# 0xPARC/plonkathon

Measured on NVIDIA H100. Metric: plonk_proofs_per_s_2^20_gates, higher is better.
Workload: dtype u256 (BN254 Fr/Fq integers, 8x32-bit Montgomery limbs)

## Files before the change

### include/plonk_b200.h

```cpp
#ifndef PLONK_B200_H
#define PLONK_B200_H
#include <stddef.h>
#include <stdint.h>

#ifdef __cplusplus
extern "C" {
#endif

typedef struct pb200_ctx pb200_ctx;
typedef struct pb200_srs pb200_srs;
typedef struct pb200_prover pb200_prover;
typedef struct pb200_transcript pb200_transcript;

const char* pb200_last_error(void);
const char* pb200_version(void);
int pb200_ctx_create(int device, void* cuda_stream, pb200_ctx** out);
void pb200_ctx_destroy(pb200_ctx* ctx);
int pb200_ctx_sync(pb200_ctx* ctx);
uint64_t pb200_ctx_launches(pb200_ctx* ctx);
int pb200_ctx_timing(pb200_ctx* ctx, int enable);
int pb200_ctx_timing_read(pb200_ctx* ctx, int category, double* total_ms, uint64_t* count);
void* pb200_ctx_stream(pb200_ctx* ctx);

int pb200_fr_to_mont(pb200_ctx* ctx, const void* d_in, void* d_out, uint64_t n);
int pb200_fr_from_mont(pb200_ctx* ctx, const void* d_in, void* d_out, uint64_t n);

int pb200_fr_vec_op(pb200_ctx* ctx, int op, const void* d_a, const void* d_b, const uint8_t* h_scalar, void* d_out,
                    uint64_t n, uint64_t shift);

int pb200_fr_ntt(pb200_ctx* ctx, const void* d_in, void* d_out, unsigned log_n, int inverse);
int pb200_fr_ntt_host(pb200_ctx* ctx, const uint8_t* h_in, uint8_t* h_out, unsigned log_n, int inverse);

int pb200_fr_ntt_decimated(pb200_ctx* ctx, const void* d_in, void* d_out, unsigned log_m, int inverse, uint64_t stride,
                           uint64_t offset);

int pb200_fr_coset_extend(pb200_ctx* ctx, const void* d_in, void* d_out, unsigned log_n, const uint8_t* h_offset);
int pb200_fr_coset_extend_host(pb200_ctx* ctx, const uint8_t* h_in, uint8_t* h_out, unsigned log_n,
                               const uint8_t* h_offset);
int pb200_fr_coset_to_coeffs(pb200_ctx* ctx, const void* d_in, void* d_out, unsigned log_n, const uint8_t* h_offset);
int pb200_fr_coset_to_coeffs_host(pb200_ctx* ctx, const uint8_t* h_in, uint8_t* h_out, unsigned log_n,
                                  const uint8_t* h_offset);
int pb200_fr_barycentric_eval(pb200_ctx* ctx, const void* d_vals, unsigned log_n, const uint8_t* h_x, uint8_t* h_out);
int pb200_fr_barycentric_eval_host(pb200_ctx* ctx, const uint8_t* h_vals, unsigned log_n, const uint8_t* h_x,
                                   uint8_t* h_out);

int pb200_g1_msm(pb200_ctx* ctx, const void* d_points, const void* d_scalars, uint64_t n, uint8_t* h_out_xy,
                 int* is_identity);
int pb200_g1_msm_host(pb200_ctx* ctx, const uint8_t* h_points, const uint8_t* h_scalars, uint64_t n,
                      uint8_t* h_out_xy, int* is_identity);

int pb200_srs_create(pb200_ctx* ctx, const uint8_t* h_points, uint64_t n, int precompute, pb200_srs** out);
int pb200_srs_generate(pb200_ctx* ctx, const uint8_t* h_tau, uint64_t n, int precompute, pb200_srs** out);
int pb200_srs_generate_lagrange(pb200_ctx* ctx, const uint8_t* h_tau, uint64_t n, int precompute, pb200_srs** out);
int pb200_srs_export(pb200_ctx* ctx, pb200_srs* srs, uint8_t* h_points, uint64_t first, uint64_t count);
void pb200_srs_destroy(pb200_srs* srs);
uint64_t pb200_srs_size(pb200_srs* srs);
int pb200_srs_commit_lagrange(pb200_ctx* ctx, pb200_srs* srs, const void* d_values, unsigned log_n,
                              uint8_t* h_out_xy, int* is_identity);
int pb200_srs_commit_lagrange_host(pb200_ctx* ctx, pb200_srs* srs, const uint8_t* h_values, unsigned log_n,
                                   uint8_t* h_out_xy, int* is_identity);
int pb200_srs_commit_coeffs(pb200_ctx* ctx, pb200_srs* srs, const void* d_coeffs, uint64_t m, int coeffs_montgomery,
                            uint8_t* h_out_xy, int* is_identity);
int pb200_srs_commit_coeffs_host(pb200_ctx* ctx, pb200_srs* srs, const uint8_t* h_coeffs, uint64_t m,
                                 uint8_t* h_out_xy, int* is_identity);

int pb200_prover_create(pb200_ctx* ctx, pb200_srs* srs, unsigned log_n, const uint8_t* const* h_pk,
                        pb200_prover** out);
int pb200_prover_create_custom(pb200_ctx* ctx, pb200_srs* srs, unsigned log_n, const uint8_t* const* h_pk,
                               unsigned n_custom, const uint8_t* h_exps, const uint8_t* const* h_custom,
                               pb200_prover** out);
void pb200_prover_destroy(pb200_prover* p);
int pb200_prover_prove(pb200_prover* p, const uint8_t* h_A, const uint8_t* h_B, const uint8_t* h_C,
                       const uint8_t* h_public, uint64_t n_public, uint8_t* h_proof768);
int pb200_prover_prove_device(pb200_prover* p, const void* d_A, const void* d_B, const void* d_C,
                              const uint8_t* h_public, uint64_t n_public, uint8_t* h_proof768);
int pb200_prover_round1(pb200_prover* p, const uint8_t* h_A, const uint8_t* h_B, const uint8_t* h_C,
                        const uint8_t* h_public, uint64_t n_public, uint8_t* h_abc_xy );
int pb200_prover_round2(pb200_prover* p, const uint8_t* beta, const uint8_t* gamma, uint8_t* h_z_xy);
int pb200_prover_round3(pb200_prover* p, const uint8_t* alpha, const uint8_t* fft_cofactor,
                        uint8_t* h_t_xy );
int pb200_prover_round4(pb200_prover* p, const uint8_t* zeta, uint8_t* h_evals );
int pb200_prover_round5(pb200_prover* p, const uint8_t* v, uint8_t* h_w_xy );

int pb200_prover_read_vector(pb200_prover* p, int which, void* d_out);
int pb200_prover_set_zk(pb200_prover* p, int enable, const uint8_t* h_blinders);
int pb200_prover_serialize(pb200_prover* p, uint8_t* h_proof768);

int pb200_prover_set_lookup(pb200_prover* p, const uint8_t* h_qk, const uint8_t* h_t1, const uint8_t* h_t2,
                            const uint8_t* h_t3, uint64_t table_rows);
int pb200_prover_round_lookup(pb200_prover* p, const uint8_t* eta, uint8_t* h_fh_xy );
int pb200_prover_round2_lookup(pb200_prover* p, const uint8_t* beta, const uint8_t* gamma, const uint8_t* delta,
                               const uint8_t* epsilon, uint8_t* h_zz2_xy );
int pb200_prover_round4_lookup(pb200_prover* p, const uint8_t* zeta, uint8_t* h_evals );
int pb200_prover_prove_lookup(pb200_prover* p, const uint8_t* h_A, const uint8_t* h_B, const uint8_t* h_C,
                              const uint8_t* h_public, uint64_t n_public, uint8_t* h_proof1216);
int pb200_prover_serialize_lookup(pb200_prover* p, uint8_t* h_proof1216);

int pb200_comm_unique_id(uint8_t* out128);
int pb200_comm_init(pb200_ctx* ctx, const uint8_t* id128, int rank, int world);
int pb200_comm_info(pb200_ctx* ctx, int* rank, int* world, uint64_t* collectives, uint64_t* bytes_received);
int pb200_fr_ntt_sharded(pb200_ctx* ctx, const void* d_in, void* d_out, unsigned log_n, int inverse);
int pb200_srs_commit_coeffs_sharded(pb200_ctx* ctx, pb200_srs* srs, const void* d_coeffs, uint64_t m,
                                    int coeffs_montgomery, uint8_t* h_out_xy, int* is_identity);
int pb200_prover_create_sharded(pb200_ctx* ctx, pb200_srs* srs, unsigned log_n, const uint8_t* const* h_pk,
                                pb200_prover** out);
int pb200_prover_create_custom_sharded(pb200_ctx* ctx, pb200_srs* srs, unsigned log_n, const uint8_t* const* h_pk,
                                       unsigned n_custom, const uint8_t* h_exps, const uint8_t* const* h_custom,
                                       pb200_prover** out);
int pb200_srs_commit_partial(pb200_ctx* ctx, pb200_srs* srs, const void* d_coeffs, uint64_t first, uint64_t count,
                             uint32_t bucket_lo, uint32_t bucket_hi, int coeffs_montgomery, uint8_t* h_xyzz128);
int pb200_srs_bucket_count(pb200_srs* srs, uint32_t* out);
int pb200_g1_combine_partials_host(const uint8_t* h_xyzz, unsigned count, uint8_t* h_out_xy, int* is_identity);
int pb200_g1_join_bucket_shards_host(const uint8_t* h_sr, unsigned world, unsigned sets, uint32_t nloc, uint8_t* h_out_xy,
                                     int* is_identity);

int pb200_transcript_create(const uint8_t* label, size_t label_len, pb200_transcript** out);
void pb200_transcript_destroy(pb200_transcript* t);
int pb200_transcript_append_message(pb200_transcript* t, const uint8_t* label, size_t label_len,
                                    const uint8_t* msg, size_t msg_len);
int pb200_transcript_challenge_bytes(pb200_transcript* t, const uint8_t* label, size_t label_len, uint8_t* out,
                                     size_t n);
int pb200_transcript_get_and_append_challenge(pb200_transcript* t, const uint8_t* label, size_t label_len,
                                              uint8_t* out_le32);

int pb200_pairing_check(const uint8_t* h_g1, const uint8_t* h_g1_identity, const uint8_t* h_g2,
                        const uint8_t* h_g2_identity, unsigned count, int* ok);
int pb200_g2_mul(const uint8_t* h_point, const uint8_t* h_scalar_le32, uint8_t* h_out, int* is_identity);
int pb200_g2_add(const uint8_t* h_p, int p_identity, const uint8_t* h_q, int q_identity, uint8_t* h_out,
                 int* is_identity);

int pb200_bench_modmul(pb200_ctx* ctx, int field , uint64_t threads, uint32_t iters, float* ms_out);

#ifdef __cplusplus
}
#endif
#endif
```

### plonkathon_b200/_lib.py

```python
from __future__ import annotations

import ctypes
import os
import threading

_HERE = os.path.dirname(os.path.abspath(__file__))
LIB_PATH = os.environ.get("PB200_LIB") or os.path.join(_HERE, "libplonk_b200.so")

c_u8p = ctypes.POINTER(ctypes.c_uint8)


class PlonkB200Error(RuntimeError):
    pass


def _load():
    if not os.path.exists(LIB_PATH):
        raise PlonkB200Error(
            "libplonk_b200.so is not built (%s); run `python -c 'import __graft_entry__ as g; g.build()'`"
            % LIB_PATH)
    lib = ctypes.CDLL(LIB_PATH)
    V, I, U, U64 = ctypes.c_void_p, ctypes.c_int, ctypes.c_uint, ctypes.c_uint64
    P = ctypes.POINTER
    sig = {
        "pb200_last_error": (ctypes.c_char_p, []),
        "pb200_version": (ctypes.c_char_p, []),
        "pb200_ctx_create": (I, [I, V, P(V)]),
        "pb200_ctx_destroy": (None, [V]),
        "pb200_ctx_sync": (I, [V]),
        "pb200_ctx_launches": (U64, [V]),
        "pb200_ctx_stream": (V, [V]),
        "pb200_ctx_timing": (I, [V, I]),
        "pb200_ctx_timing_read": (I, [V, I, P(ctypes.c_double), P(U64)]),
        "pb200_fr_to_mont": (I, [V, V, V, U64]),
        "pb200_fr_from_mont": (I, [V, V, V, U64]),
        "pb200_fr_ntt": (I, [V, V, V, U, I]),
        "pb200_fr_ntt_host": (I, [V, V, V, U, I]),
        "pb200_fr_ntt_decimated": (I, [V, V, V, U, I, U64, U64]),
        "pb200_fr_ntt_sharded": (I, [V, V, V, U, I]),
        "pb200_fr_vec_op": (I, [V, I, V, V, V, V, U64, U64]),
        "pb200_prover_read_vector": (I, [V, I, V]),
        "pb200_comm_unique_id": (I, [V]),
        "pb200_comm_init": (I, [V, V, I, I]),
        "pb200_comm_info": (I, [V, P(I), P(I), P(U64), P(U64)]),
        "pb200_srs_commit_coeffs_sharded": (I, [V, V, V, U64, I, V, P(I)]),
        "pb200_prover_create_sharded": (I, [V, V, U, V, P(V)]),
        "pb200_srs_commit_partial": (I, [V, V, V, U64, U64, U, U, I, V]),
        "pb200_srs_bucket_count": (I, [V, P(U)]),
        "pb200_g1_join_bucket_shards_host": (I, [V, U, U, U, V, P(I)]),
        "pb200_fr_coset_extend": (I, [V, V, V, U, V]),
        "pb200_fr_coset_extend_host": (I, [V, V, V, U, V]),
        "pb200_fr_coset_to_coeffs": (I, [V, V, V, U, V]),
        "pb200_fr_coset_to_coeffs_host": (I, [V, V, V, U, V]),
        "pb200_fr_barycentric_eval": (I, [V, V, U, V, V]),
        "pb200_fr_barycentric_eval_host": (I, [V, V, U, V, V]),
        "pb200_g1_msm": (I, [V, V, V, U64, V, P(I)]),
        "pb200_g1_msm_host": (I, [V, V, V, U64, V, P(I)]),
        "pb200_srs_create": (I, [V, V, U64, I, P(V)]),
        "pb200_srs_generate": (I, [V, V, U64, I, P(V)]),
        "pb200_srs_generate_lagrange": (I, [V, V, U64, I, P(V)]),
        "pb200_srs_export": (I, [V, V, V, U64, U64]),
        "pb200_srs_destroy": (None, [V]),
        "pb200_srs_size": (U64, [V]),
        "pb200_srs_commit_lagrange": (I, [V, V, V, U, V, P(I)]),
        "pb200_srs_commit_lagrange_host": (I, [V, V, V, U, V, P(I)]),
        "pb200_srs_commit_coeffs_host": (I, [V, V, V, U64, V, P(I)]),
        "pb200_srs_commit_coeffs": (I, [V, V, V, U64, I, V, P(I)]),
        "pb200_prover_create": (I, [V, V, U, V, P(V)]),
        "pb200_prover_create_custom": (I, [V, V, U, V, U, V, V, P(V)]),
        "pb200_prover_create_custom_sharded": (I, [V, V, U, V, U, V, V, P(V)]),
        "pb200_prover_destroy": (None, [V]),
        "pb200_prover_prove": (I, [V, V, V, V, V, U64, V]),
        "pb200_prover_prove_device": (I, [V, V, V, V, V, U64, V]),
        "pb200_prover_round1": (I, [V, V, V, V, V, U64, V]),
        "pb200_prover_round2": (I, [V, V, V, V]),
        "pb200_prover_round3": (I, [V, V, V, V]),
        "pb200_prover_round4": (I, [V, V, V]),
        "pb200_prover_round5": (I, [V, V, V]),
        "pb200_prover_serialize": (I, [V, V]),
        "pb200_prover_set_zk": (I, [V, I, V]),
        "pb200_prover_set_lookup": (I, [V, V, V, V, V, U64]),
        "pb200_prover_round_lookup": (I, [V, V, V]),
        "pb200_prover_round2_lookup": (I, [V, V, V, V, V, V]),
        "pb200_prover_round4_lookup": (I, [V, V, V]),
        "pb200_prover_prove_lookup": (I, [V, V, V, V, V, U64, V]),
        "pb200_prover_serialize_lookup": (I, [V, V]),
        "pb200_g1_combine_partials_host": (I, [V, U, V, P(I)]),
        "pb200_transcript_create": (I, [V, ctypes.c_size_t, P(V)]),
        "pb200_transcript_destroy": (None, [V]),
        "pb200_transcript_append_message": (I, [V, V, ctypes.c_size_t, V, ctypes.c_size_t]),
        "pb200_transcript_challenge_bytes": (I, [V, V, ctypes.c_size_t, V, ctypes.c_size_t]),
        "pb200_transcript_get_and_append_challenge": (I, [V, V, ctypes.c_size_t, V]),
        "pb200_pairing_check": (I, [V, V, V, V, U, P(I)]),
        "pb200_g2_mul": (I, [V, V, V, P(I)]),
        "pb200_g2_add": (I, [V, I, V, I, V, P(I)]),
        "pb200_bench_modmul": (I, [V, I, U64, U, P(ctypes.c_float)]),
    }
    for name, (res, args) in sig.items():
        fn = getattr(lib, name)
        fn.restype = res
        fn.argtypes = args
    return lib, tuple(sig)


_lock = threading.Lock()
_lib = None
EXPORTS = ()


def lib():
    global _lib, EXPORTS
    with _lock:
        if _lib is None:
            _lib, EXPORTS = _load()
    return _lib


def check(rc):
    if rc != 0:
        raise PlonkB200Error(lib().pb200_last_error().decode())


class Context:

    def __init__(self, device: int = 0, stream: int | None = None):
        h = ctypes.c_void_p()
        check(lib().pb200_ctx_create(device, ctypes.c_void_p(stream), ctypes.byref(h)))
        self.handle = h
        self.device = device

    def sync(self):
        check(lib().pb200_ctx_sync(self.handle))

    @property
    def launches(self) -> int:
        return int(lib().pb200_ctx_launches(self.handle))

    @property
    def stream(self) -> int:
        return int(lib().pb200_ctx_stream(self.handle) or 0)

    def close(self):
        if self.handle:
            lib().pb200_ctx_destroy(self.handle)
            self.handle = None

    def __del__(self):
        try:
            self.close()
        except Exception:
            pass


_default_ctx = None


def default_context() -> Context:
    global _default_ctx
    if _default_ctx is None:
        _default_ctx = Context(int(os.environ.get("LOCAL_RANK", "0")))
    return _default_ctx
```

### plonkathon_b200/csrc/capi.cu

```cuda
#include "../../include/plonk_b200.h"

#include <cstring>

#include "common.cuh"
#include "comm.cuh"
#include "msm_bucket.cuh"
#include "prover.cuh"
#include "pairing.cuh"
#include "transcript.cuh"

namespace pb200 {
void ntt_run(Context* ctx, const Fr* in, Fr* out, int log_n, bool inverse, uint64_t n_in, const Fr* in_scale,
             const Fr* out_scale);
void launch_powers(Context* ctx, Fr* out, uint64_t n, const Fr& base, const Fr& scale);
Fr fr_from_u64(uint64_t x);
void ntt_run_strided(Context* ctx, const Fr* in, Fr* out, int log_n, bool inverse, uint64_t n_in,
                     const Fr* in_scale, const Fr* out_scale, uint64_t in_mul, uint64_t in_add);
void ntt_sharded(Context* ctx, const Fr* const* in, Fr* const* out, int count, int log_n, bool inverse);
void fr_to_mont(Context* ctx, const Fr* in, Fr* out, uint64_t n);
void fr_from_mont(Context* ctx, const Fr* in, Fr* out, uint64_t n);
void fr_vec_op(Context* ctx, int op, const Fr* a, const Fr* b, const Fr& scalar_canonical, Fr* out, uint64_t n,
               uint64_t shift);
void barycentric_eval(Context* ctx, const Fr* d_vals, int log_n, const Fr& x_mont, Fr* h_out);
float bench_modmul(Context* ctx, int field, uint64_t threads, uint32_t iters);
struct Srs;
Srs* srs_create(Context* ctx, const uint8_t* h_points, uint64_t n, int precompute);
void srs_destroy(Srs* s);
Srs* srs_generate(Context* ctx, const Fr& tau_canonical, uint64_t n, int precompute);
Srs* srs_generate_lagrange(Context* ctx, const Fr& tau_canonical, uint64_t n, int precompute);
void srs_export(Context* ctx, Srs* srs, uint8_t* h_points, uint64_t first, uint64_t count);
void srs_msm(Context* ctx, Srs* srs, const Fr* d_scalars, uint64_t m, bool scalars_mont, uint8_t* out_xy, int* is_identity);
uint64_t srs_size(Srs* s);
uint32_t msm_default_window(uint64_t n, bool fixed_base);
void msm_run(Context* ctx, const G1Affine* points, uint64_t n, const Fr* scalars, bool scalars_mont, uint32_t c,
             bool fixed_base, uint64_t point_stride, uint8_t* out_xy, int* is_identity);
void affine_to_mont(Context* ctx, const G1Affine* in, G1Affine* out, uint64_t n);
Prover* prover_create(Context* ctx, Srs* srs, int log_n, const uint8_t* const* h_pk, int n_custom,
                      const uint8_t* h_exps, const uint8_t* const* h_custom, bool sharded);
void prover_destroy(Prover* p);
void prover_prove(Prover* P, const uint8_t* hA, const uint8_t* hB, const uint8_t* hC, const uint8_t* h_public,
                  uint64_t n_public, uint8_t* out768, bool wires_on_device);
void prover_round1(Prover* P, const uint8_t* hA, const uint8_t* hB, const uint8_t* hC, const uint8_t* h_public,
                   uint64_t n_public, bool wires_on_device);
void prover_round2(Prover* P, const Fr& beta_c, const Fr& gamma_c);
void prover_round3(Prover* P, const Fr& alpha_c, const Fr& cofactor_c);
void prover_round4(Prover* P, const Fr& zeta_c);
void prover_round5(Prover* P, const Fr& v_c);
void prover_serialize(const Prover* P, uint8_t* out768);
void prover_set_zk(Prover* P, bool enable, const uint8_t* h_blinders);
void prover_set_lookup(Prover* P, const uint8_t* h_qk, const uint8_t* const* h_tab, uint64_t rows);
void prover_round_lookup(Prover* P, const Fr& eta_c);
void prover_round2_lookup(Prover* P, const Fr& beta_c, const Fr& gamma_c, const Fr& delta_c, const Fr& epsilon_c);
void prover_round4_lookup(Prover* P, const Fr& zeta_c);
void prover_prove_lookup(Prover* P, const uint8_t* hA, const uint8_t* hB, const uint8_t* hC, const uint8_t* h_public,
                         uint64_t n_public, uint8_t* out1216);
void prover_serialize_lookup(const Prover* P, uint8_t* out1216);
void g1_combine_partials_host(const G1XYZZ* parts, uint32_t count, uint8_t* out_xy, int* is_identity);
void host_join_bucket_shards(const SR* all, uint32_t world, uint32_t sets, uint32_t nloc, G1XYZZ* out);
void host_join_bucket_shards_strided(const SR* all, uint32_t world, uint32_t sets, G1XYZZ* out);
}

using namespace pb200;

static thread_local std::string g_err;

#define PB_API_BEGIN try {
#define PB_API_END                        \
  return 0;                               \
  }                                       \
  catch (const std::exception& e) {       \
    g_err = e.what();                     \
    return 1;                             \
  }                                       \
  catch (...) {                           \
    g_err = "unknown error";              \
    return 1;                             \
  }

static Context* C(pb200_ctx* c) { return reinterpret_cast<Context*>(c); }

#define PB_NOT_LOOKUP(P, entry)                                                                       \
  PB_CHECK(!(P)->lk, "this prover has a lookup argument: its proofs have 1216 bytes; use " entry)

struct DeviceGuard {
  int prev = -1;
  explicit DeviceGuard(const Context* c) {
    int cur = -1;
    cudaGetDevice(&cur);
    if (cur != c->device) { cudaSetDevice(c->device); prev = cur; }
  }
  ~DeviceGuard() { if (prev >= 0) cudaSetDevice(prev); }
};
#define PB_ON_CTX(c) DeviceGuard guard__(c)

static Fr load_fr_canonical(const uint8_t* h) {
  Fr a;
  memcpy(a.v, h, 32);
  Fr m = Fr::modulus();
  bool lt = false;
  for (int i = 7; i >= 0; i--) {
    if (a.v[i] != m.v[i]) { lt = a.v[i] < m.v[i]; break; }
  }
  PB_CHECK(lt, "Fr value not reduced below the modulus");
  return a;
}

extern "C" {

const char* pb200_last_error(void) { return g_err.c_str(); }
const char* pb200_version(void) { return "plonk_b200 0.1 (sm_90a)"; }

int pb200_ctx_create(int device, void* cuda_stream, pb200_ctx** out) {
  PB_API_BEGIN
  int count = 0;
  cudaError_t e = cudaGetDeviceCount(&count);
  PB_CHECK(e == cudaSuccess && count > 0, "no CUDA device: libplonk_b200 has no CPU fallback");
  PB_CHECK(device >= 0 && device < count, "bad device ordinal");
  PB_CUDA(cudaSetDevice(device));
  auto ctx = std::make_unique<Context>();
  ctx->device = device;
  cudaDeviceProp prop;
  PB_CUDA(cudaGetDeviceProperties(&prop, device));
  ctx->sm_count = prop.multiProcessorCount;
  if (cuda_stream) {
    ctx->stream = reinterpret_cast<cudaStream_t>(cuda_stream);
  } else {
    PB_CUDA(cudaStreamCreateWithFlags(&ctx->stream, cudaStreamNonBlocking));
    ctx->own_stream = true;
  }
  *out = reinterpret_cast<pb200_ctx*>(ctx.release());
  PB_API_END
}

void pb200_ctx_destroy(pb200_ctx* ctx) {
  if (!ctx) return;
  cudaSetDevice(C(ctx)->device);
  cudaStreamSynchronize(C(ctx)->stream);
  delete C(ctx);
}

int pb200_ctx_sync(pb200_ctx* ctx) {
  PB_API_BEGIN PB_ON_CTX(C(ctx));
  PB_CUDA(cudaStreamSynchronize(C(ctx)->stream));
  PB_API_END
}

uint64_t pb200_ctx_launches(pb200_ctx* ctx) { return C(ctx)->launches; }

int pb200_ctx_timing(pb200_ctx* ctx, int enable) {
  PB_API_BEGIN PB_ON_CTX(C(ctx));
  Context* c = C(ctx);
  PB_CUDA(cudaStreamSynchronize(c->stream));
  for (auto& v : c->timed) {
    for (auto& pr : v) { cudaEventDestroy(pr.first); cudaEventDestroy(pr.second); }
    v.clear();
  }
  c->timing = enable != 0;
  PB_API_END
}
int pb200_ctx_timing_read(pb200_ctx* ctx, int category, double* total_ms, uint64_t* count) {
  PB_API_BEGIN PB_ON_CTX(C(ctx));
  Context* c = C(ctx);
  PB_CHECK(category >= 0 && category < 4, "bad timing category");
  PB_CUDA(cudaStreamSynchronize(c->stream));
  double t = 0;
  for (auto& pr : c->timed[category]) {
    float ms = 0;
    PB_CUDA(cudaEventElapsedTime(&ms, pr.first, pr.second));
    t += ms;
  }
  *total_ms = t;
  *count = c->timed[category].size();
  PB_API_END
}
void* pb200_ctx_stream(pb200_ctx* ctx) { return (void*)C(ctx)->stream; }

int pb200_fr_to_mont(pb200_ctx* ctx, const void* d_in, void* d_out, uint64_t n) {
  PB_API_BEGIN PB_ON_CTX(C(ctx));
  fr_to_mont(C(ctx), (const Fr*)d_in, (Fr*)d_out, n);
  PB_API_END
}
int pb200_fr_from_mont(pb200_ctx* ctx, const void* d_in, void* d_out, uint64_t n) {
  PB_API_BEGIN PB_ON_CTX(C(ctx));
  fr_from_mont(C(ctx), (const Fr*)d_in, (Fr*)d_out, n);
  PB_API_END
}

int pb200_fr_vec_op(pb200_ctx* ctx, int op, const void* d_a, const void* d_b, const uint8_t* h_scalar, void* d_out,
                    uint64_t n, uint64_t shift) {
  PB_API_BEGIN PB_ON_CTX(C(ctx));
  Fr s = Fr::zero();
  if (h_scalar) s = load_fr_canonical(h_scalar);
  PB_CHECK(op < 4 ? d_b != nullptr : true, "missing second operand");
  fr_vec_op(C(ctx), op, (const Fr*)d_a, (const Fr*)d_b, s, (Fr*)d_out, n, shift);
  PB_API_END
}

int pb200_fr_ntt(pb200_ctx* ctx, const void* d_in, void* d_out, unsigned log_n, int inverse) {
  PB_API_BEGIN PB_ON_CTX(C(ctx));
  ntt_run(C(ctx), (const Fr*)d_in, (Fr*)d_out, (int)log_n, inverse != 0, (uint64_t)1 << log_n, nullptr, nullptr);
  PB_API_END
}

int pb200_fr_ntt_decimated(pb200_ctx* ctx, const void* d_in, void* d_out, unsigned log_m, int inverse, uint64_t stride,
                           uint64_t offset) {
  PB_API_BEGIN PB_ON_CTX(C(ctx));
  PB_CHECK(stride >= 1, "bad stride");
  ntt_run_strided(C(ctx), (const Fr*)d_in, (Fr*)d_out, (int)log_m, inverse != 0, (uint64_t)1 << log_m, nullptr, nullptr,
                  stride, offset);
  PB_API_END
}
int pb200_fr_ntt_sharded(pb200_ctx* ctx, const void* d_in, void* d_out, unsigned log_n, int inverse) {
  PB_API_BEGIN PB_ON_CTX(C(ctx));
  const Fr* in = (const Fr*)d_in;
  Fr* out = (Fr*)d_out;
  ntt_sharded(C(ctx), &in, &out, 1, (int)log_n, inverse != 0);
  PB_API_END
}

int pb200_comm_unique_id(uint8_t* out128) {
  PB_API_BEGIN
  comm_unique_id(out128);
  PB_API_END
}
int pb200_comm_init(pb200_ctx* ctx, const uint8_t* id128, int rank, int world) {
  PB_API_BEGIN PB_ON_CTX(C(ctx));
  Context* c = C(ctx);
  PB_CHECK(!c->comm, "this context already has a communicator");
  c->comm = comm_create(id128, rank, world);
  PB_API_END
}
int pb200_comm_info(pb200_ctx* ctx, int* rank, int* world, uint64_t* collectives, uint64_t* bytes_received) {
  PB_API_BEGIN
  Context* c = C(ctx);
  *rank = c->comm ? c->comm->rank : 0;
  *world = c->comm ? c->comm->world : 1;
  *collectives = c->comm ? c->comm->collectives : 0;
  *bytes_received = c->comm ? c->comm->bytes_gathered : 0;
  PB_API_END
}

struct HostStage {
  Context* ctx;
  DevBuf in, out;
  HostStage(Context* c, const uint8_t* h_in, size_t in_bytes, size_t out_bytes) : ctx(c), in(in_bytes), out(out_bytes) {
    if (in_bytes) PB_CUDA(cudaMemcpyAsync(in.p, h_in, in_bytes, cudaMemcpyHostToDevice, ctx->stream));
  }
  void finish(uint8_t* h_out, size_t bytes) {
    PB_CUDA(cudaMemcpyAsync(h_out, out.p, bytes, cudaMemcpyDeviceToHost, ctx->stream));
    PB_CUDA(cudaStreamSynchronize(ctx->stream));
  }
};

int pb200_fr_ntt_host(pb200_ctx* ctx, const uint8_t* h_in, uint8_t* h_out, unsigned log_n, int inverse) {
  PB_API_BEGIN PB_ON_CTX(C(ctx));
  size_t bytes = ((size_t)1 << log_n) * 32;
  HostStage st(C(ctx), h_in, bytes, bytes);
  ntt_run(C(ctx), st.in.as<Fr>(), st.out.as<Fr>(), (int)log_n, inverse != 0, (uint64_t)1 << log_n, nullptr, nullptr);
  st.finish(h_out, bytes);
  PB_API_END
}

static void coset_extend(Context* ctx, const Fr* d_in, Fr* d_out, int log_n, const uint8_t* h_offset) {
  uint64_t n = (uint64_t)1 << log_n;
  Fr off = fp_to_mont(load_fr_canonical(h_offset));
  DevBuf coeffs(n * 32), powers(n * 32);
  ntt_run(ctx, d_in, coeffs.as<Fr>(), log_n, true, n, nullptr, nullptr);
  launch_powers(ctx, powers.as<Fr>(), n, off, Fr::one());
  ntt_run(ctx, coeffs.as<Fr>(), d_out, log_n + 2, false, n, powers.as<Fr>(), nullptr);
  PB_CUDA(cudaStreamSynchronize(ctx->stream));
}

static void coset_to_coeffs(Context* ctx, const Fr* d_in, Fr* d_out, int log_n, const uint8_t* h_offset) {
  uint64_t n = (uint64_t)1 << log_n;
  Fr off = fp_to_mont(load_fr_canonical(h_offset));
  Fr inv = fp_inv(off);
  DevBuf powers(n * 32);
  launch_powers(ctx, powers.as<Fr>(), n, inv, Fr::one());
  ntt_run(ctx, d_in, d_out, log_n, true, n, nullptr, powers.as<Fr>());
  PB_CUDA(cudaStreamSynchronize(ctx->stream));
}

int pb200_fr_coset_extend(pb200_ctx* ctx, const void* d_in, void* d_out, unsigned log_n, const uint8_t* h_offset) {
  PB_API_BEGIN PB_ON_CTX(C(ctx));
  coset_extend(C(ctx), (const Fr*)d_in, (Fr*)d_out, (int)log_n, h_offset);
  PB_API_END
}
int pb200_fr_coset_extend_host(pb200_ctx* ctx, const uint8_t* h_in, uint8_t* h_out, unsigned log_n,
                               const uint8_t* h_offset) {
  PB_API_BEGIN PB_ON_CTX(C(ctx));
  size_t bytes = ((size_t)1 << log_n) * 32;
  HostStage st(C(ctx), h_in, bytes, bytes * 4);
  coset_extend(C(ctx), st.in.as<Fr>(), st.out.as<Fr>(), (int)log_n, h_offset);
  st.finish(h_out, bytes * 4);
  PB_API_END
}
int pb200_fr_coset_to_coeffs(pb200_ctx* ctx, const void* d_in, void* d_out, unsigned log_n, const uint8_t* h_offset) {
  PB_API_BEGIN PB_ON_CTX(C(ctx));
  coset_to_coeffs(C(ctx), (const Fr*)d_in, (Fr*)d_out, (int)log_n, h_offset);
  PB_API_END
}
int pb200_fr_coset_to_coeffs_host(pb200_ctx* ctx, const uint8_t* h_in, uint8_t* h_out, unsigned log_n,
                                  const uint8_t* h_offset) {
  PB_API_BEGIN PB_ON_CTX(C(ctx));
  size_t bytes = ((size_t)1 << log_n) * 32;
  HostStage st(C(ctx), h_in, bytes, bytes);
  coset_to_coeffs(C(ctx), st.in.as<Fr>(), st.out.as<Fr>(), (int)log_n, h_offset);
  st.finish(h_out, bytes);
  PB_API_END
}

int pb200_fr_barycentric_eval(pb200_ctx* ctx, const void* d_vals, unsigned log_n, const uint8_t* h_x, uint8_t* h_out) {
  PB_API_BEGIN PB_ON_CTX(C(ctx));
  Fr x = fp_to_mont(load_fr_canonical(h_x));
  Fr r;
  barycentric_eval(C(ctx), (const Fr*)d_vals, (int)log_n, x, &r);
  memcpy(h_out, r.v, 32);
  PB_API_END
}
int pb200_fr_barycentric_eval_host(pb200_ctx* ctx, const uint8_t* h_vals, unsigned log_n, const uint8_t* h_x,
                                   uint8_t* h_out) {
  PB_API_BEGIN PB_ON_CTX(C(ctx));
  size_t bytes = ((size_t)1 << log_n) * 32;
  HostStage st(C(ctx), h_vals, bytes, 0);
  Fr x = fp_to_mont(load_fr_canonical(h_x));
  Fr r;
  barycentric_eval(C(ctx), st.in.as<Fr>(), (int)log_n, x, &r);
  memcpy(h_out, r.v, 32);
  PB_API_END
}

int pb200_g1_msm(pb200_ctx* ctx, const void* d_points, const void* d_scalars, uint64_t n, uint8_t* h_out_xy,
                 int* is_identity) {
  PB_API_BEGIN PB_ON_CTX(C(ctx));
  PB_CHECK(n > 0, "ec_lincomb of an empty list (the reference raises ValueError, curve.py:93)");
  Context* c = C(ctx);
  DevBuf mont(n * sizeof(G1Affine));
  affine_to_mont(c, (const G1Affine*)d_points, mont.as<G1Affine>(), n);
  msm_run(c, mont.as<G1Affine>(), n, (const Fr*)d_scalars, false, msm_default_window(n, false), false, 0, h_out_xy,
          is_identity);
  PB_API_END
}

int pb200_g1_msm_host(pb200_ctx* ctx, const uint8_t* h_points, const uint8_t* h_scalars, uint64_t n,
                      uint8_t* h_out_xy, int* is_identity) {
  PB_API_BEGIN PB_ON_CTX(C(ctx));
  PB_CHECK(n > 0, "ec_lincomb of an empty list (the reference raises ValueError, curve.py:93)");
  Context* c = C(ctx);
  DevBuf pts(n * 64), sc(n * 32);
  PB_CUDA(cudaMemcpyAsync(pts.p, h_points, n * 64, cudaMemcpyHostToDevice, c->stream));
  PB_CUDA(cudaMemcpyAsync(sc.p, h_scalars, n * 32, cudaMemcpyHostToDevice, c->stream));
  int rc = pb200_g1_msm(ctx, pts.p, sc.p, n, h_out_xy, is_identity);
  if (rc) throw Error(g_err);
  PB_API_END
}

int pb200_srs_create(pb200_ctx* ctx, const uint8_t* h_points, uint64_t n, int precompute, pb200_srs** out) {
  PB_API_BEGIN PB_ON_CTX(C(ctx));
  PB_CHECK(n > 0, "empty SRS");
  *out = reinterpret_cast<pb200_srs*>(srs_create(C(ctx), h_points, n, precompute));
  PB_API_END
}
int pb200_srs_generate(pb200_ctx* ctx, const uint8_t* h_tau, uint64_t n, int precompute, pb200_srs** out) {
  PB_API_BEGIN PB_ON_CTX(C(ctx));
  PB_CHECK(n > 0, "empty SRS");
  *out = reinterpret_cast<pb200_srs*>(srs_generate(C(ctx), load_fr_canonical(h_tau), n, precompute));
  PB_API_END
}
int pb200_srs_generate_lagrange(pb200_ctx* ctx, const uint8_t* h_tau, uint64_t n, int precompute, pb200_srs** out) {
  PB_API_BEGIN PB_ON_CTX(C(ctx));
  PB_CHECK(n > 0, "empty SRS");
  *out = reinterpret_cast<pb200_srs*>(srs_generate_lagrange(C(ctx), load_fr_canonical(h_tau), n, precompute));
  PB_API_END
}
int pb200_srs_commit_coeffs_host(pb200_ctx* ctx, pb200_srs* srs, const uint8_t* h_coeffs, uint64_t m,
                                 uint8_t* h_out_xy, int* is_identity) {
  PB_API_BEGIN PB_ON_CTX(C(ctx));
  HostStage st(C(ctx), h_coeffs, (size_t)m * 32, 0);
  srs_msm(C(ctx), reinterpret_cast<Srs*>(srs), (const Fr*)st.in.p, m, false, h_out_xy, is_identity);
  PB_API_END
}
int pb200_srs_export(pb200_ctx* ctx, pb200_srs* srs, uint8_t* h_points, uint64_t first, uint64_t count) {
  PB_API_BEGIN PB_ON_CTX(C(ctx));
  srs_export(C(ctx), reinterpret_cast<Srs*>(srs), h_points, first, count);
  PB_API_END
}
void pb200_srs_destroy(pb200_srs* srs) { srs_destroy(reinterpret_cast<Srs*>(srs)); }
uint64_t pb200_srs_size(pb200_srs* srs) { return srs_size(reinterpret_cast<Srs*>(srs)); }

int pb200_srs_commit_lagrange(pb200_ctx* ctx, pb200_srs* srs, const void* d_values, unsigned log_n, uint8_t* h_out_xy,
                              int* is_identity) {
  PB_API_BEGIN PB_ON_CTX(C(ctx));
  Context* c = C(ctx);
  uint64_t n = (uint64_t)1 << log_n;
  PB_CHECK(n <= srs_size(reinterpret_cast<Srs*>(srs)), "Not enough powers in setup");
  DevBuf coeffs(n * 32);
  ntt_run(c, (const Fr*)d_values, coeffs.as<Fr>(), (int)log_n, true, n, nullptr, nullptr);
  srs_msm(c, reinterpret_cast<Srs*>(srs), coeffs.as<Fr>(), n, false, h_out_xy, is_identity);
  PB_API_END
}
int pb200_srs_commit_lagrange_host(pb200_ctx* ctx, pb200_srs* srs, const uint8_t* h_values, unsigned log_n,
                                   uint8_t* h_out_xy, int* is_identity) {
  PB_API_BEGIN PB_ON_CTX(C(ctx));
  size_t bytes = ((size_t)1 << log_n) * 32;
  HostStage st(C(ctx), h_values, bytes, 0);
  int rc = pb200_srs_commit_lagrange(ctx, srs, st.in.p, log_n, h_out_xy, is_identity);
  if (rc) throw Error(g_err);
  PB_API_END
}
int pb200_srs_commit_coeffs(pb200_ctx* ctx, pb200_srs* srs, const void* d_coeffs, uint64_t m, int coeffs_montgomery,
                            uint8_t* h_out_xy, int* is_identity) {
  PB_API_BEGIN PB_ON_CTX(C(ctx));
  srs_msm(C(ctx), reinterpret_cast<Srs*>(srs), (const Fr*)d_coeffs, m, coeffs_montgomery != 0, h_out_xy, is_identity);
  PB_API_END
}

int pb200_prover_create(pb200_ctx* ctx, pb200_srs* srs, unsigned log_n, const uint8_t* const* h_pk,
                        pb200_prover** out) {
  return pb200_prover_create_custom(ctx, srs, log_n, h_pk, 0, nullptr, nullptr, out);
}
int pb200_prover_create_sharded(pb200_ctx* ctx, pb200_srs* srs, unsigned log_n, const uint8_t* const* h_pk,
                                pb200_prover** out) {
  return pb200_prover_create_custom_sharded(ctx, srs, log_n, h_pk, 0, nullptr, nullptr, out);
}
int pb200_prover_create_custom(pb200_ctx* ctx, pb200_srs* srs, unsigned log_n, const uint8_t* const* h_pk,
                               unsigned n_custom, const uint8_t* h_exps, const uint8_t* const* h_custom,
                               pb200_prover** out) {
  PB_API_BEGIN PB_ON_CTX(C(ctx));
  *out = reinterpret_cast<pb200_prover*>(prover_create(C(ctx), reinterpret_cast<Srs*>(srs), (int)log_n, h_pk,
                                                       (int)n_custom, h_exps, h_custom, false));
  PB_API_END
}
int pb200_prover_create_custom_sharded(pb200_ctx* ctx, pb200_srs* srs, unsigned log_n, const uint8_t* const* h_pk,
                                       unsigned n_custom, const uint8_t* h_exps, const uint8_t* const* h_custom,
                                       pb200_prover** out) {
  PB_API_BEGIN PB_ON_CTX(C(ctx));
  *out = reinterpret_cast<pb200_prover*>(prover_create(C(ctx), reinterpret_cast<Srs*>(srs), (int)log_n, h_pk,
                                                       (int)n_custom, h_exps, h_custom, true));
  PB_API_END
}
void pb200_prover_destroy(pb200_prover* p) { prover_destroy(reinterpret_cast<Prover*>(p)); }

int pb200_prover_prove(pb200_prover* p, const uint8_t* h_A, const uint8_t* h_B, const uint8_t* h_C,
                       const uint8_t* h_public, uint64_t n_public, uint8_t* h_proof768) {
  PB_API_BEGIN PB_ON_CTX(reinterpret_cast<Prover*>(p)->ctx);
  PB_NOT_LOOKUP(reinterpret_cast<Prover*>(p), "pb200_prover_prove_lookup");
  prover_prove(reinterpret_cast<Prover*>(p), h_A, h_B, h_C, h_public, n_public, h_proof768, false);
  PB_API_END
}
int pb200_prover_prove_device(pb200_prover* p, const void* d_A, const void* d_B, const void* d_C,
                              const uint8_t* h_public, uint64_t n_public, uint8_t* h_proof768) {
  PB_API_BEGIN PB_ON_CTX(reinterpret_cast<Prover*>(p)->ctx);
  PB_NOT_LOOKUP(reinterpret_cast<Prover*>(p), "pb200_prover_prove_lookup (wires in host memory)");
  prover_prove(reinterpret_cast<Prover*>(p), (const uint8_t*)d_A, (const uint8_t*)d_B, (const uint8_t*)d_C, h_public,
               n_public, h_proof768, true);
  PB_API_END
}
int pb200_prover_round1(pb200_prover* p, const uint8_t* h_A, const uint8_t* h_B, const uint8_t* h_C,
                        const uint8_t* h_public, uint64_t n_public, uint8_t* h_abc_xy) {
  PB_API_BEGIN PB_ON_CTX(reinterpret_cast<Prover*>(p)->ctx);
  Prover* P = reinterpret_cast<Prover*>(p);
  prover_round1(P, h_A, h_B, h_C, h_public, n_public, false);
  memcpy(h_abc_xy, P->proof.pts[0], 3 * 64);
  PB_API_END
}
int pb200_prover_round2(pb200_prover* p, const uint8_t* beta, const uint8_t* gamma, uint8_t* h_z_xy) {
  PB_API_BEGIN PB_ON_CTX(reinterpret_cast<Prover*>(p)->ctx);
  Prover* P = reinterpret_cast<Prover*>(p);
  PB_NOT_LOOKUP(P, "pb200_prover_round2_lookup");
  prover_round2(P, load_fr_canonical(beta), load_fr_canonical(gamma));
  memcpy(h_z_xy, P->proof.pts[3], 64);
  PB_API_END
}
int pb200_prover_round3(pb200_prover* p, const uint8_t* alpha, const uint8_t* fft_cofactor, uint8_t* h_t_xy) {
  PB_API_BEGIN PB_ON_CTX(reinterpret_cast<Prover*>(p)->ctx);
  Prover* P = reinterpret_cast<Prover*>(p);
  prover_round3(P, load_fr_canonical(alpha), load_fr_canonical(fft_cofactor));
  memcpy(h_t_xy, P->proof.pts[4], 3 * 64);
  PB_API_END
}
int pb200_prover_round4(pb200_prover* p, const uint8_t* zeta, uint8_t* h_evals) {
  PB_API_BEGIN PB_ON_CTX(reinterpret_cast<Prover*>(p)->ctx);
  Prover* P = reinterpret_cast<Prover*>(p);
  PB_NOT_LOOKUP(P, "pb200_prover_round4_lookup");
  prover_round4(P, load_fr_canonical(zeta));
  memcpy(h_evals, P->proof.evals[0], 6 * 32);
  PB_API_END
}
int pb200_prover_round5(pb200_prover* p, const uint8_t* v, uint8_t* h_w_xy) {
  PB_API_BEGIN PB_ON_CTX(reinterpret_cast<Prover*>(p)->ctx);
  Prover* P = reinterpret_cast<Prover*>(p);
  prover_round5(P, load_fr_canonical(v));
  memcpy(h_w_xy, P->proof.pts[7], 2 * 64);
  PB_API_END
}

int pb200_prover_read_vector(pb200_prover* p, int which, void* d_out) {
  PB_API_BEGIN PB_ON_CTX(reinterpret_cast<Prover*>(p)->ctx);
  Prover* P = reinterpret_cast<Prover*>(p);
  const Fr* src = nullptr;
  switch (which) {
    case 0: case 1: case 2: case 3: src = P->lag[which].as<Fr>(); break;
    case 4: src = P->pi_lag.as<Fr>(); break;
    case 5: case 6: case 7:
      PB_CHECK(!P->zk, "T1, T2, T3 are not n-coefficient vectors in zero-knowledge mode (the blinded pieces have n + 1, "
                       "n + 1 and n + 6 coefficients)");
      src = P->tq.as<Fr>() + (uint64_t)(which - 5) * P->n;
      break;
    default: PB_CHECK(false, "unknown prover vector");
  }
  fr_from_mont(P->ctx, src, (Fr*)d_out, P->n);
  PB_CUDA(cudaStreamSynchronize(P->ctx->stream));
  PB_API_END
}
int pb200_prover_set_zk(pb200_prover* p, int enable, const uint8_t* h_blinders) {
  PB_API_BEGIN PB_ON_CTX(reinterpret_cast<Prover*>(p)->ctx);
  prover_set_zk(reinterpret_cast<Prover*>(p), enable != 0, h_blinders);
  PB_API_END
}
int pb200_prover_serialize(pb200_prover* p, uint8_t* h_proof768) {
  PB_API_BEGIN PB_ON_CTX(reinterpret_cast<Prover*>(p)->ctx);
  PB_NOT_LOOKUP(reinterpret_cast<Prover*>(p), "pb200_prover_serialize_lookup");
  prover_serialize(reinterpret_cast<Prover*>(p), h_proof768);
  PB_API_END
}
int pb200_prover_set_lookup(pb200_prover* p, const uint8_t* h_qk, const uint8_t* h_t1, const uint8_t* h_t2,
                            const uint8_t* h_t3, uint64_t table_rows) {
  PB_API_BEGIN PB_ON_CTX(reinterpret_cast<Prover*>(p)->ctx);
  const uint8_t* tab[3] = {h_t1, h_t2, h_t3};
  prover_set_lookup(reinterpret_cast<Prover*>(p), h_qk, tab, table_rows);
  PB_API_END
}
int pb200_prover_round_lookup(pb200_prover* p, const uint8_t* eta, uint8_t* h_fh_xy) {
  PB_API_BEGIN PB_ON_CTX(reinterpret_cast<Prover*>(p)->ctx);
  Prover* P = reinterpret_cast<Prover*>(p);
  prover_round_lookup(P, load_fr_canonical(eta));
  memcpy(h_fh_xy, P->lk_pts[0], 3 * 64);
  PB_API_END
}
int pb200_prover_round2_lookup(pb200_prover* p, const uint8_t* beta, const uint8_t* gamma, const uint8_t* delta,
                               const uint8_t* epsilon, uint8_t* h_zz2_xy) {
  PB_API_BEGIN PB_ON_CTX(reinterpret_cast<Prover*>(p)->ctx);
  Prover* P = reinterpret_cast<Prover*>(p);
  prover_round2_lookup(P, load_fr_canonical(beta), load_fr_canonical(gamma), load_fr_canonical(delta),
                       load_fr_canonical(epsilon));
  memcpy(h_zz2_xy, P->proof.pts[3], 64);
  memcpy(h_zz2_xy + 64, P->lk_pts[3], 64);
  PB_API_END
}
int pb200_prover_round4_lookup(pb200_prover* p, const uint8_t* zeta, uint8_t* h_evals) {
  PB_API_BEGIN PB_ON_CTX(reinterpret_cast<Prover*>(p)->ctx);
  Prover* P = reinterpret_cast<Prover*>(p);
  prover_round4_lookup(P, load_fr_canonical(zeta));
  memcpy(h_evals, P->proof.evals[0], 6 * 32);
  memcpy(h_evals + 6 * 32, P->lk_evals[0], 6 * 32);
  PB_API_END
}
int pb200_prover_prove_lookup(pb200_prover* p, const uint8_t* h_A, const uint8_t* h_B, const uint8_t* h_C,
                              const uint8_t* h_public, uint64_t n_public, uint8_t* h_proof1216) {
  PB_API_BEGIN PB_ON_CTX(reinterpret_cast<Prover*>(p)->ctx);
  prover_prove_lookup(reinterpret_cast<Prover*>(p), h_A, h_B, h_C, h_public, n_public, h_proof1216);
  PB_API_END
}
int pb200_prover_serialize_lookup(pb200_prover* p, uint8_t* h_proof1216) {
  PB_API_BEGIN PB_ON_CTX(reinterpret_cast<Prover*>(p)->ctx);
  Prover* P = reinterpret_cast<Prover*>(p);
  PB_CHECK(P->lk, "this prover has no lookup table: use pb200_prover_serialize (768 bytes)");
  prover_serialize_lookup(P, h_proof1216);
  PB_API_END
}
int pb200_g1_combine_partials_host(const uint8_t* h_xyzz, unsigned count, uint8_t* h_out_xy, int* is_identity) {
  PB_API_BEGIN
  std::vector<G1XYZZ> parts(count);
  memcpy(parts.data(), h_xyzz, (size_t)count * sizeof(G1XYZZ));
  g1_combine_partials_host(parts.data(), count, h_out_xy, is_identity);
  PB_API_END
}

int pb200_srs_commit_partial(pb200_ctx* ctx, pb200_srs* srs, const void* d_coeffs, uint64_t first, uint64_t count,
                             uint32_t bucket_lo, uint32_t bucket_hi, int coeffs_montgomery, uint8_t* h_xyzz128) {
  PB_API_BEGIN PB_ON_CTX(C(ctx));
  const Fr* sc = (const Fr*)d_coeffs;
  G1XYZZ part;
  srs_msm_batch_partial(C(ctx), reinterpret_cast<Srs*>(srs), &sc, 1, first, count, bucket_lo, bucket_hi,
                        coeffs_montgomery != 0, &part);
  memcpy(h_xyzz128, &part, sizeof(part));
  PB_API_END
}
int pb200_srs_bucket_count(pb200_srs* srs, uint32_t* out) {
  PB_API_BEGIN
  *out = srs_bucket_count(reinterpret_cast<Srs*>(srs));
  PB_API_END
}
int pb200_srs_commit_coeffs_sharded(pb200_ctx* ctx, pb200_srs* srs, const void* d_coeffs, uint64_t m,
                                    int coeffs_montgomery, uint8_t* h_out_xy, int* is_identity) {
  PB_API_BEGIN PB_ON_CTX(C(ctx));
  const Fr* sc = (const Fr*)d_coeffs;
  srs_msm_batch_sharded(C(ctx), reinterpret_cast<Srs*>(srs), &sc, 1, m, coeffs_montgomery != 0, h_out_xy, is_identity);
  PB_API_END
}
int pb200_g1_join_bucket_shards_host(const uint8_t* h_sr, unsigned world, unsigned sets, uint32_t nloc, uint8_t* h_out_xy,
                                     int* is_identity) {
  PB_API_BEGIN
  std::vector<SR> all((size_t)world * sets);
  memcpy(all.data(), h_sr, all.size() * sizeof(SR));
  std::vector<G1XYZZ> ws(sets);
  if (nloc == 0) host_join_bucket_shards_strided(all.data(), world, sets, ws.data());
  else host_join_bucket_shards(all.data(), world, sets, nloc, ws.data());
  for (unsigned k = 0; k < sets; k++) g1_combine_partials_host(&ws[k], 1, h_out_xy + 64 * k, is_identity + k);
  PB_API_END
}

int pb200_transcript_create(const uint8_t* label, size_t label_len, pb200_transcript** out) {
  PB_API_BEGIN
  *out = reinterpret_cast<pb200_transcript*>(new Transcript(std::string((const char*)label, label_len)));
  PB_API_END
}
void pb200_transcript_destroy(pb200_transcript* t) { delete reinterpret_cast<Transcript*>(t); }
int pb200_transcript_append_message(pb200_transcript* t, const uint8_t* label, size_t label_len, const uint8_t* msg,
                                    size_t msg_len) {
  PB_API_BEGIN
  reinterpret_cast<Transcript*>(t)->append_message(std::string((const char*)label, label_len), msg, msg_len);
  PB_API_END
}
int pb200_transcript_challenge_bytes(pb200_transcript* t, const uint8_t* label, size_t label_len, uint8_t* out,
                                     size_t n) {
  PB_API_BEGIN
  reinterpret_cast<Transcript*>(t)->challenge_bytes(std::string((const char*)label, label_len), out, n);
  PB_API_END
}
int pb200_transcript_get_and_append_challenge(pb200_transcript* t, const uint8_t* label, size_t label_len,
                                              uint8_t* out_le32) {
  PB_API_BEGIN
  Fr f = reinterpret_cast<Transcript*>(t)->get_and_append_challenge(std::string((const char*)label, label_len));
  memcpy(out_le32, f.v, 32);
  PB_API_END
}

static Fq load_fq_canonical(const uint8_t* h) {
  Fq a;
  memcpy(a.v, h, 32);
  Fq m = Fq::modulus();
  bool lt = false;
  for (int i = 7; i >= 0; i--) {
    if (a.v[i] != m.v[i]) { lt = a.v[i] < m.v[i]; break; }
  }
  PB_CHECK(lt, "Fq value not reduced below the modulus");
  return fp_to_mont(a);
}
static G2Affine load_g2(const uint8_t* h, bool inf) {
  G2Affine q;
  q.inf = inf;
  q.x = {load_fq_canonical(h), load_fq_canonical(h + 32)};
  q.y = {load_fq_canonical(h + 64), load_fq_canonical(h + 96)};
  PB_CHECK(inf || g2_on_curve(q), "G2 point is not on the twist curve");
  return q;
}
static void store_g2(const G2Affine& q, uint8_t* out, int* is_identity) {
  *is_identity = q.inf ? 1 : 0;
  memset(out, 0, 128);
  if (q.inf) return;
  const Fq c[4] = {fp_from_mont(q.x.a), fp_from_mont(q.x.b), fp_from_mont(q.y.a), fp_from_mont(q.y.b)};
  for (int k = 0; k < 4; k++) memcpy(out + 32 * k, c[k].v, 32);
}
static const Bn254Pairing& pairing_engine() {
  static const Bn254Pairing engine;
  return engine;
}

int pb200_pairing_check(const uint8_t* h_g1, const uint8_t* h_g1_identity, const uint8_t* h_g2,
                        const uint8_t* h_g2_identity, unsigned count, int* ok) {
  PB_API_BEGIN
  std::vector<G1Host> ps(count);
  std::vector<G2Affine> qs(count);
  const Fq three = fq_small(3);
  for (unsigned i = 0; i < count; i++) {
    ps[i].inf = h_g1_identity && h_g1_identity[i];
    if (!ps[i].inf) {
      ps[i].x = load_fq_canonical(h_g1 + 64 * i);
      ps[i].y = load_fq_canonical(h_g1 + 64 * i + 32);
      PB_CHECK(fp_sqr(ps[i].y) == fp_add(fp_mul(fp_sqr(ps[i].x), ps[i].x), three), "G1 point is not on the curve");
    }
    qs[i] = load_g2(h_g2 + 128 * i, h_g2_identity && h_g2_identity[i]);
  }
  *ok = pairing_engine().product_is_one(ps, qs) ? 1 : 0;
  PB_API_END
}
int pb200_g2_mul(const uint8_t* h_point, const uint8_t* h_scalar_le32, uint8_t* h_out, int* is_identity) {
  PB_API_BEGIN
  G2Affine p = load_g2(h_point, false);
  uint32_t k[8];
  memcpy(k, h_scalar_le32, 32);
  store_g2(g2_mul(p, k), h_out, is_identity);
  PB_API_END
}
int pb200_g2_add(const uint8_t* h_p, int p_identity, const uint8_t* h_q, int q_identity, uint8_t* h_out,
                 int* is_identity) {
  PB_API_BEGIN
  store_g2(g2_add(load_g2(h_p, p_identity != 0), load_g2(h_q, q_identity != 0)), h_out, is_identity);
  PB_API_END
}

int pb200_bench_modmul(pb200_ctx* ctx, int field, uint64_t threads, uint32_t iters, float* ms_out) {
  PB_API_BEGIN PB_ON_CTX(C(ctx));
  *ms_out = bench_modmul(C(ctx), field, threads, iters);
  PB_API_END
}

}
```

### plonkathon_b200/csrc/host_selftest.cpp

```cpp
#include "field.cuh"
#include "curve.cuh"
#include "msm_digits.cuh"
#include "modinv.cuh"
#include "msm_bucket.cuh"
#include "msm_sort.cuh"
#include "ntt_shard.cuh"
#include <algorithm>
#include <vector>
#include <cstring>
using namespace pb200;

template <class F> static F ld(const uint32_t* p) { F r; memcpy(r.v, p, 32); return r; }
template <class F> static void st(uint32_t* p, const F& a) { memcpy(p, a.v, 32); }

extern "C" {
int hs_field_op(int field, int op, const uint32_t* a, const uint32_t* b, uint32_t* out) {
#define RUN(F)                                                   \
  {                                                              \
    F x = ld<F>(a), y = ld<F>(b), r;                             \
    switch (op) {                                                \
      case 0: r = fp_add(x, y); break;                           \
      case 1: r = fp_sub(x, y); break;                           \
      case 2: r = fp_mul(x, y); break;                           \
      case 3: r = fp_neg(x); break;                              \
      case 4: r = fp_inv(x); break;                              \
      case 5: r = fp_to_mont(x); break;                          \
      case 6: r = fp_from_mont(x); break;                        \
      case 7: r = fp_dbl(x); break;                              \
      case 8: r = fp_sqr(x); break;                              \
      case 9: r = fp_inv_gcd(x); break;                          \
      case 10: r = fp_inv_plain_gcd(x); break;                   \
      case 11: r = fp_mul_lazy(x, y); break;                     \
      case 12: r = fp_sqr_lazy(x); break;                        \
      case 13: r = fp_sub_lazy(x, y); break;                     \
      case 14: r = fp_neg_lazy(x); break;                        \
      case 15: r = fp_is_zero_lazy(x) ? F::one() : F::zero(); break; \
      default: return -1;                                        \
    }                                                            \
    st(out, r);                                                  \
  }
  if (field == 0) RUN(Fr) else RUN(Fq)
#undef RUN
  return 0;
}

int hs_field_mul2(int field, const uint32_t* a, const uint32_t* b, const uint32_t* c, const uint32_t* d, uint32_t* out) {
  if (field == 0) st(out, fp_mul2_lazy(ld<Fr>(a), ld<Fr>(b), ld<Fr>(c), ld<Fr>(d)));
  else st(out, fp_mul2_lazy(ld<Fq>(a), ld<Fq>(b), ld<Fq>(c), ld<Fq>(d)));
  return 0;
}
}

static Fq ref_sqr(const Fq& a) { return fp_mul(a, a); }
static void ref_double(G1XYZZ& a) {
  if (a.is_inf()) return;
  Fq U = fp_dbl(a.Y), V = ref_sqr(U), W = fp_mul(U, V), S = fp_mul(a.X, V), M = ref_sqr(a.X);
  M = fp_add(fp_dbl(M), M);
  Fq X3 = fp_sub(ref_sqr(M), fp_dbl(S));
  a.Y = fp_sub(fp_mul(M, fp_sub(S, X3)), fp_mul(W, a.Y));
  a.X = X3;
  a.ZZ = fp_mul(V, a.ZZ);
  a.ZZZ = fp_mul(W, a.ZZZ);
}
static void ref_add_mixed(G1XYZZ& acc, const G1Affine& p) {
  if (acc.is_inf()) { acc = g1_from_affine(p); return; }
  Fq U2 = fp_mul(p.x, acc.ZZ), S2 = fp_mul(p.y, acc.ZZZ), Pd = fp_sub(U2, acc.X), Rd = fp_sub(S2, acc.Y);
  if (Pd.is_zero()) {
    if (Rd.is_zero()) { acc = g1_from_affine(p); ref_double(acc); }
    else acc = G1XYZZ::identity();
    return;
  }
  Fq PP = ref_sqr(Pd), PPP = fp_mul(Pd, PP), Q = fp_mul(acc.X, PP);
  Fq X3 = fp_sub(fp_sub(ref_sqr(Rd), PPP), fp_dbl(Q));
  acc.Y = fp_sub(fp_mul(Rd, fp_sub(Q, X3)), fp_mul(acc.Y, PPP));
  acc.X = X3;
  acc.ZZ = fp_mul(acc.ZZ, PP);
  acc.ZZZ = fp_mul(acc.ZZZ, PPP);
}
static void ref_add(G1XYZZ& acc, const G1XYZZ& q) {
  if (q.is_inf()) return;
  if (acc.is_inf()) { acc = q; return; }
  Fq U1 = fp_mul(acc.X, q.ZZ), U2 = fp_mul(q.X, acc.ZZ), S1 = fp_mul(acc.Y, q.ZZZ), S2 = fp_mul(q.Y, acc.ZZZ);
  Fq Pd = fp_sub(U2, U1), Rd = fp_sub(S2, S1);
  if (Pd.is_zero()) {
    if (Rd.is_zero()) ref_double(acc);
    else acc = G1XYZZ::identity();
    return;
  }
  Fq PP = ref_sqr(Pd), PPP = fp_mul(Pd, PP), Q = fp_mul(U1, PP);
  Fq X3 = fp_sub(fp_sub(ref_sqr(Rd), PPP), fp_dbl(Q));
  acc.Y = fp_sub(fp_mul(Rd, fp_sub(Q, X3)), fp_mul(S1, PPP));
  acc.X = X3;
  acc.ZZ = fp_mul(fp_mul(acc.ZZ, q.ZZ), PP);
  acc.ZZZ = fp_mul(fp_mul(acc.ZZZ, q.ZZZ), PPP);
}

extern "C" {
int hs_curve_op_ref(int op, const uint32_t* acc_in, const uint32_t* other, int other_inf, uint32_t* out) {
  G1XYZZ acc;
  memcpy(&acc, acc_in, sizeof(acc));
  if (op == 0 || op == 4) {
    G1Affine p;
    memcpy(&p.x, other, 32);
    memcpy(&p.y, other + 8, 32);
    if (!other_inf) ref_add_mixed(acc, p);
  } else if (op == 1 || op == 5) {
    G1XYZZ q;
    memcpy(&q, other, sizeof(q));
    ref_add(acc, q);
  } else if (op == 2) {
    ref_double(acc);
  } else {
    return -1;
  }
  memcpy(out, &acc, sizeof(acc));
  return 0;
}

int hs_small_dft(int log_g, const uint32_t* x, const uint32_t* tw, uint32_t* out) {
  DftTw t;
  for (int k = 0; k < 4; k++) t.w[k] = ld<Fr>(tw + 8 * k);
#define RUN_DFT(LG)                                                     \
  {                                                                     \
    Fr v[1 << LG];                                                      \
    for (int i = 0; i < (1 << LG); i++) v[i] = ld<Fr>(x + 8 * i);       \
    small_dft<LG>(v, t);                                                \
    for (int i = 0; i < (1 << LG); i++) st(out + 8 * i, v[i]);          \
  }
  switch (log_g) {
    case 1: RUN_DFT(1) break;
    case 2: RUN_DFT(2) break;
    case 3: RUN_DFT(3) break;
    default: return -1;
  }
#undef RUN_DFT
  return 0;
}

int hs_msm_digits(const uint32_t* scalar, uint32_t c, int32_t* digits, uint32_t* n_windows) {
  MsmGeom g;
  g.c = c;
  g.W = (256 + c - 1) / c;
  g.half = 1u << (c - 1);
  g.fixed_base = 0;
  g.point_stride = 0;
  g.batch = 1;
  g.lo = 0;
  g.nloc = g.half;
  g.own_log = 0;
  g.own_rank = 0;
  g.sets = g.W;
  g.nb = g.half * g.W;
  Fr s = ld<Fr>(scalar);
  DigitWalk dw(&s, 0, 0);
  for (uint32_t w = 0; w < g.W; w++) {
    uint32_t neg, d = dw.next(w, g, neg);
    digits[w] = neg ? -(int32_t)d : (int32_t)d;
  }
  *n_windows = g.W;
  return (int)dw.carry;
}

int hs_curve_op(int op, const uint32_t* acc_in, const uint32_t* other, int other_inf, uint32_t* out) {
  G1XYZZ acc;
  memcpy(&acc, acc_in, sizeof(acc));
  switch (op) {
    case 0: {
      G1Affine p;
      memcpy(&p.x, other, 32);
      memcpy(&p.y, other + 8, 32);
      if (!other_inf) g1_add_mixed(acc, p);
      break;
    }
    case 4: {
      G1Affine p;
      memcpy(&p.x, other, 32);
      memcpy(&p.y, other + 8, 32);
      if (!other_inf) g1_add_mixed_uniform(acc, p);
      break;
    }
    case 1: {
      G1XYZZ q;
      memcpy(&q, other, sizeof(q));
      g1_add(acc, q);
      break;
    }
    case 2: g1_double(acc); break;
    case 5: {
      G1XYZZ q;
      memcpy(&q, other, sizeof(q));
      g1_add_uniform(acc, q);
      break;
    }
    case 3: {
      G1Affine p;
      bool inf = g1_to_affine(acc, p);
      memcpy(out, &p.x, 32);
      memcpy(out + 8, &p.y, 32);
      return inf ? 1 : 0;
    }
    default: return -1;
  }
  memcpy(out, &acc, sizeof(acc));
  return 0;
}

}

static bool msm_geom(uint32_t n, uint32_t batch, uint32_t c, int fixed_base, uint32_t lo, uint32_t hi, MsmGeom& g) {
  g.c = c;
  g.W = (256 + c - 1) / c;
  g.half = 1u << (c - 1);
  g.fixed_base = fixed_base ? 1 : 0;
  g.point_stride = fixed_base ? n : 0;
  g.batch = batch;
  g.own_log = 0;
  g.own_rank = 0;
  if (hi >= 0xfffffff0u && hi != 0xffffffffu) {
    g.own_log = 0xffffffffu - hi;
    g.own_rank = lo;
    g.lo = 0;
    g.nloc = g.half >> g.own_log;
    if (!g.nloc || lo >= (1u << g.own_log)) return false;
  } else {
    if (hi > g.half) hi = g.half;
    if (lo >= hi) return false;
    g.lo = lo;
    g.nloc = hi - lo;
  }
  g.sets = fixed_base ? batch : g.W;
  g.nb = g.sets * g.nloc;
  return true;
}

static void host_scan(uint32_t* cnt, uint32_t len, uint32_t pad, uint32_t* off, uint32_t* max_out) {
  uint32_t run = 0, m = 0;
  for (uint32_t b = 0; b < len; b++) {
    off[b] = run;
    run += (cnt[b] + pad) & ~pad;
    m = std::max(m, cnt[b]);
    cnt[b] = 0;
  }
  off[len] = run;
  if (max_out) *max_out = m;
}

static void host_msm_sort(const MsmGeom& g, const std::vector<Fr>& sc, uint32_t n, uint32_t pad, uint32_t lb,
                          uint32_t T, uint32_t spb, uint32_t bin_nt, uint32_t chunk_nt, std::vector<uint32_t>& counts,
                          std::vector<uint32_t>& off, std::vector<uint32_t>& sorted) {
  const uint32_t nbins = ((g.nb - 1) >> lb) + 1;
  const uint32_t batch = g.fixed_base ? g.batch : 1;
  std::vector<uint32_t> bin_cnt(nbins, 0), bin_off(nbins + 1), chunk_first(nbins + 1);
  std::vector<SortEntry> binned((size_t)n * g.W * batch);
  counts.assign(g.nb + 1, 0);
  off.assign(g.nb + 1, 0);
  SortArgs a;
  for (uint32_t k = 0; k < 4; k++) a.sb.p[k] = k < batch ? sc.data() + (size_t)k * n : nullptr;
  a.n = n;
  a.from_mont = 0;
  a.g = g;
  a.lb = lb;
  a.nbins = nbins;
  a.T = T;
  a.bin_cnt = bin_cnt.data();
  a.bin_off = bin_off.data();
  a.binned = binned.data();
  a.chunk_first = chunk_first.data();
  a.counts = counts.data();
  a.offsets = off.data();
  a.sorted = nullptr;
  a.spb = spb;
  std::vector<uint32_t> sh_cnt(std::max(nbins, 1u << lb)), sh_loc(sh_cnt.size()), sh_base(sh_cnt.size()), runs;
  std::vector<SortEntry> bin_stage_buf((size_t)spb * g.W);
  std::vector<uint32_t> chunk_stage_buf(T);
  auto block_scan = [&](uint32_t len, uint32_t nt) {
    runs.assign(nt, 0);
    uint32_t run = 0;
    for (uint32_t t = 0; t < nt; t++) { runs[t] = run; run += scan_part_sum(sh_cnt.data(), len, t, nt); }
    return run;
  };
  const uint32_t bin_blocks = (n + spb - 1) / spb;
  for (uint32_t k = 0; k < batch; k++)
    for (uint32_t bx = 0; bx < bin_blocks; bx++) {
      for (uint32_t t = 0; t < bin_nt; t++) sort_zero(sh_cnt.data(), nbins, t, bin_nt);
      for (uint32_t t = 0; t < bin_nt; t++) bin_hist(a, bx, k, t, bin_nt, sh_cnt.data());
      for (uint32_t t = 0; t < bin_nt; t++) bin_flush(a, t, bin_nt, sh_cnt.data());
    }
  host_scan(bin_cnt.data(), nbins, 0, bin_off.data(), nullptr);
  for (uint32_t k = batch; k-- > 0;)
    for (uint32_t bx = bin_blocks; bx-- > 0;) {
      for (uint32_t t = 0; t < bin_nt; t++) sort_zero(sh_cnt.data(), nbins, t, bin_nt);
      for (uint32_t t = 0; t < bin_nt; t++) bin_hist(a, bx, k, t, bin_nt, sh_cnt.data());
      const uint32_t total = block_scan(nbins, bin_nt);
      for (uint32_t t = 0; t < bin_nt; t++)
        bin_reserve(a, t, bin_nt, runs[t], sh_cnt.data(), sh_loc.data(), sh_base.data());
      for (uint32_t t = 0; t < bin_nt; t++) bin_stage(a, bx, k, t, bin_nt, sh_cnt.data(), sh_loc.data(), bin_stage_buf.data());
      for (uint32_t t = 0; t < bin_nt; t++)
        bin_copy_out(a, t, bin_nt, total, sh_loc.data(), sh_base.data(), bin_stage_buf.data());
    }
  {
    std::vector<uint32_t> sums(256);
    for (uint32_t t = 0; t < 256; t++) sums[t] = chunk_map_sum(a, t);
    uint32_t run = 0;
    for (uint32_t t = 0; t < 256; t++) { const uint32_t s = sums[t]; sums[t] = run; run += s; }
    for (uint32_t t = 0; t < 256; t++) chunk_map_write(a, t, sums[t], run);
  }
  const uint32_t grid = 3;
  SortChunk ch;
  for (uint32_t bx = 0; bx < grid; bx++)
    for (uint32_t c = bx; chunk_locate(a, c, ch); c += grid) {
      for (uint32_t t = 0; t < chunk_nt; t++) sort_zero(sh_cnt.data(), ch.nkeys, t, chunk_nt);
      for (uint32_t t = 0; t < chunk_nt; t++) chunk_hist(a, ch, t, chunk_nt, sh_cnt.data());
      for (uint32_t t = 0; t < chunk_nt; t++) chunk_flush(a, ch, t, chunk_nt, sh_cnt.data());
    }
  host_scan(counts.data(), g.nb, pad, off.data(), &counts[g.nb]);
  sorted.assign(off[g.nb] + 2, PB_MSM_PAD);
  a.sorted = sorted.data();
  for (uint32_t bx = grid; bx-- > 0;)
    for (uint32_t c = bx; chunk_locate(a, c, ch); c += grid) {
      for (uint32_t t = 0; t < chunk_nt; t++) sort_zero(sh_cnt.data(), ch.nkeys, t, chunk_nt);
      for (uint32_t t = 0; t < chunk_nt; t++) chunk_hist(a, ch, t, chunk_nt, sh_cnt.data());
      const uint32_t total = block_scan(ch.nkeys, chunk_nt);
      for (uint32_t t = 0; t < chunk_nt; t++)
        chunk_reserve(a, ch, t, chunk_nt, runs[t], sh_cnt.data(), sh_loc.data(), sh_base.data());
      for (uint32_t t = 0; t < chunk_nt; t++) chunk_stage(a, ch, t, chunk_nt, sh_cnt.data(), sh_loc.data(), chunk_stage_buf.data());
      for (uint32_t t = 0; t < chunk_nt; t++)
        chunk_copy_out(a, ch, t, chunk_nt, sh_loc.data(), sh_base.data(), chunk_stage_buf.data());
      if (total != ch.hi - ch.lo) abort();
    }
}

extern "C" {
int hs_msm_sort(const uint32_t* scalars, uint32_t n, uint32_t batch, uint32_t c, int fixed_base, uint32_t lo,
                uint32_t hi, uint32_t pad, uint32_t lb, uint32_t T, uint32_t spb, uint32_t bin_nt, uint32_t chunk_nt,
                uint32_t* counts_out, uint32_t* off_out, uint32_t* sorted_out, uint32_t cap) {
  if (!n || !batch || batch > 4 || (!fixed_base && batch != 1) || c < 1 || c > 16 || !T || !bin_nt || !chunk_nt)
    return -1;
  MsmGeom g;
  if (!msm_geom(n, batch, c, fixed_base, lo, hi, g)) return -1;
  if (lb == 0xffffffffu) lb = sort_default_lb(g.nb);
  if (((g.nb - 1) >> lb) >= PB_SORT_MAX_BINS || (1u << lb) > PB_SORT_MAX_BIN_KEYS) return -1;
  if (!spb) spb = PB_SORT_BIN_STAGE / g.W;
  std::vector<Fr> sc((size_t)batch * n);
  for (size_t i = 0; i < sc.size(); i++) sc[i] = ld<Fr>(scalars + 8 * i);
  std::vector<uint32_t> counts, off, sorted;
  host_msm_sort(g, sc, n, pad ? 1 : 0, lb, T, spb, bin_nt, chunk_nt, counts, off, sorted);
  if (off[g.nb] > cap) return -1;
  memcpy(counts_out, counts.data(), counts.size() * 4);
  memcpy(off_out, off.data(), off.size() * 4);
  memcpy(sorted_out, sorted.data(), (size_t)off[g.nb] * 4);
  return (int)g.nb;
}

int hs_msm_pipeline(const uint32_t* points, uint32_t n, const uint32_t* scalars, uint32_t batch, uint32_t c,
                    int fixed_base, uint32_t lo, uint32_t hi, uint32_t B, uint32_t g0, uint32_t* out, uint8_t* out_inf) {
  if (!n || !batch || batch > 4 || (!fixed_base && batch != 1) || c < 1 || c > 16 || B < 2 || B > PB_AFF_BMAX) return -1;
  if (g0 < 2 || (g0 & (g0 - 1))) return -1;
  MsmGeom g;
  if (!msm_geom(n, batch, c, fixed_base, lo, hi, g)) return -1;
  std::vector<G1Affine> tab(fixed_base ? (size_t)g.W * n : n);
  for (uint32_t i = 0; i < n; i++) {
    tab[i].x = fp_to_mont(ld<Fq>(points + 16 * i));
    tab[i].y = fp_to_mont(ld<Fq>(points + 16 * i + 8));
  }
  if (fixed_base)
    for (uint32_t w = 1; w < g.W; w++)
      for (uint32_t i = 0; i < n; i++) {
        G1XYZZ a;
        g1_double_affine(a, tab[(size_t)(w - 1) * n + i]);
        for (uint32_t k = 1; k < c; k++) g1_double(a);
        g1_to_affine(a, tab[(size_t)w * n + i]);
      }
  std::vector<Fr> sc((size_t)batch * n);
  for (size_t i = 0; i < sc.size(); i++) sc[i] = ld<Fr>(scalars + 8 * i);
  std::vector<uint32_t> counts, off, sorted;
  host_msm_sort(g, sc, n, 1, sort_default_lb(g.nb), PB_SORT_CHUNK, PB_SORT_BIN_STAGE / g.W, PB_SORT_BIN_THREADS,
                PB_SORT_CHUNK_THREADS, counts, off, sorted);
  const uint32_t maxc = counts[g.nb];
  const uint64_t positions = (uint64_t)n * g.W * batch + g.nb, s_bound = positions / 2;
  std::vector<G1Affine> pts(s_bound + 1);
  AffAcc a;
  a.table = tab.data();
  a.sorted = sorted.data();
  a.pts = pts.data();
  a.off = off.data();
  a.cnt = counts.data();
  a.max_cnt = counts.data() + g.nb;
  a.nbl = g.nb;
  a.B = B;
  Fq pref[PB_AFF_BMAX];
  uint32_t desc[PB_AFF_BMAX];
  int rounds = 0;
  for (uint32_t r = 0; r < 32; r++) {
    a.r = r;
    if (r > 0 && maxc > (1u << r)) rounds = r + 1;
    if (r == 0) rounds = 1;
    const uint64_t T = aff_round_threads(s_bound, B, r) + 40;
    for (uint64_t t = T; t-- > 0;) {
      if (r == 0) aff_round0_thread(a, t, pref, desc);
      else aff_round_thread(a, t, pref, desc);
    }
  }
  ReduceArgs ra;
  ra.pts = pts.data(); ra.off = off.data(); ra.cnt = counts.data(); ra.xb = nullptr;
  ra.sets = g.sets; ra.m = g.nloc; ra.g = g0;
  std::vector<SR> cur((size_t)g.sets * reduce_groups(ra.m, ra.g)), nxt;
  ra.out = cur.data();
  for (uint64_t t = 0; t < cur.size() + 3; t++) reduce_level0_thread(ra, t);
  uint32_t m = reduce_groups(ra.m, ra.g), log_G = 0;
  while ((1u << log_G) < g0) log_G++;
  while (m > 8) {
    const uint32_t chunks = reduce_chunks(m);
    nxt.assign((size_t)g.sets * chunks, SR());
    BlockLevelArgs ba;
    ba.in = cur.data(); ba.out = nxt.data(); ba.sets = g.sets; ba.m = m; ba.log_G = log_G;
    for (uint32_t set = 0; set < g.sets; set++)
      for (uint32_t chunk = 0; chunk < chunks; chunk++) {
        const uint32_t NT = PB_REDUCE_THREADS;
        std::vector<G1XYZZ> sh(NT), xs(NT), tmp(NT);
        for (uint32_t t = 0; t < NT; t++) blk_local(ba, set, chunk, t, sh[t], xs[t]);
        for (uint32_t d = 1; d < NT; d <<= 1) {
          for (uint32_t t = 0; t < NT; t++) tmp[t] = blk_scan_step(sh.data(), t, d);
          sh = tmp;
        }
        const G1XYZZ s_total = sh[0];
        for (uint32_t t = 0; t < NT; t++) tmp[t] = blk_weight(ba, t, xs[t], sh[t]);
        sh = tmp;
        for (uint32_t d = NT / 2; d > 0; d >>= 1)
          for (uint32_t t = 0; t < NT; t++) blk_tree_step(sh.data(), t, d);
        nxt[(size_t)set * chunks + chunk].S = s_total;
        nxt[(size_t)set * chunks + chunk].R = sh[0];
      }
    m = chunks;
    log_G += 9;
    cur.swap(nxt);
  }
  {
    std::vector<SR> fin(g.sets);
    for (uint32_t s = 0; s < g.sets; s++) fin[s] = reduce_fold_final(cur.data() + (size_t)s * m, m, log_G);
    cur.swap(fin);
  }
  std::vector<G1XYZZ> ws(g.sets);
  for (uint32_t s = 0; s < g.sets; s++) {
    if (g.own_log) {
      std::vector<SR> one(1, cur[s]);
      G1XYZZ gr = cur[s].R;
      for (uint32_t k = 0; k < g.own_log; k++) g1_double(gr);
      G1XYZZ ms = G1XYZZ::identity();
      const uint32_t coef = (1u << g.own_log) - 1 - g.own_rank;
      for (int i = 31; i >= 0; i--) { g1_double(ms); if ((coef >> i) & 1) g1_add(ms, cur[s].S); }
      ms.Y = fp_neg(ms.Y);
      g1_add(gr, ms);
      ws[s] = gr;
      continue;
    }
    ws[s] = cur[s].R;
    G1XYZZ ml = G1XYZZ::identity();
    for (int i = 31; i >= 0; i--) { g1_double(ml); if ((g.lo >> i) & 1) g1_add(ml, cur[s].S); }
    g1_add(ws[s], ml);
  }
  auto emit = [&](const G1XYZZ& r, uint32_t k) {
    G1Affine p;
    bool inf = g1_to_affine(r, p);
    out_inf[k] = inf ? 1 : 0;
    Fq x = fp_from_mont(p.x), y = fp_from_mont(p.y);
    st(out + 16 * k, x);
    st(out + 16 * k + 8, y);
  };
  if (fixed_base) {
    for (uint32_t k = 0; k < batch; k++) emit(ws[k], k);
  } else {
    G1XYZZ r = G1XYZZ::identity();
    for (int w = (int)g.W - 1; w >= 0; w--) {
      if (w != (int)g.W - 1) for (uint32_t k = 0; k < c; k++) g1_double(r);
      g1_add(r, ws[w]);
    }
    emit(r, 0);
  }
  return rounds;
}
}
```

### plonkathon_b200/csrc/msm.cu

```cuda
#include <algorithm>
#include <cstring>

#include "common.cuh"
#include "comm.cuh"
#include "msm_bucket.cuh"
#include "msm_digits.cuh"
#include "msm_sort.cuh"

namespace pb200 {

__device__ __forceinline__ G1Affine ld_affine(const G1Affine* p) {
  const uint4* q = reinterpret_cast<const uint4*>(p);
  uint4 a = __ldg(q), b = __ldg(q + 1), c = __ldg(q + 2), d = __ldg(q + 3);
  G1Affine r;
  r.x.v[0] = a.x; r.x.v[1] = a.y; r.x.v[2] = a.z; r.x.v[3] = a.w;
  r.x.v[4] = b.x; r.x.v[5] = b.y; r.x.v[6] = b.z; r.x.v[7] = b.w;
  r.y.v[0] = c.x; r.y.v[1] = c.y; r.y.v[2] = c.z; r.y.v[3] = c.w;
  r.y.v[4] = d.x; r.y.v[5] = d.y; r.y.v[6] = d.z; r.y.v[7] = d.w;
  return r;
}

__device__ __forceinline__ uint32_t block_exclusive_scan(uint32_t v, uint32_t* sh, uint32_t* total) {
  const uint32_t lane = threadIdx.x & 31, wid = threadIdx.x >> 5, nw = blockDim.x >> 5;
  uint32_t x = v;
  for (int d = 1; d < 32; d <<= 1) {
    uint32_t y = __shfl_up_sync(0xffffffffu, x, d);
    if ((int)lane >= d) x += y;
  }
  if (lane == 31) sh[wid] = x;
  __syncthreads();
  if (wid == 0) {
    uint32_t w = lane < nw ? sh[lane] : 0;
    for (int d = 1; d < 32; d <<= 1) {
      uint32_t y = __shfl_up_sync(0xffffffffu, w, d);
      if ((int)lane >= d) w += y;
    }
    if (lane < nw) sh[lane] = w;
  }
  __syncthreads();
  uint32_t base = wid ? sh[wid - 1] : 0;
  *total = sh[nw - 1];
  __syncthreads();
  return base + x - v;
}

__global__ void __launch_bounds__(PB_SORT_BIN_THREADS) k_msm_bin_count(SortArgs a) {
  __shared__ uint32_t sh_cnt[PB_SORT_MAX_BINS];
  const uint32_t t = threadIdx.x, nt = blockDim.x;
  sort_zero(sh_cnt, a.nbins, t, nt);
  __syncthreads();
  bin_hist(a, blockIdx.x, blockIdx.y, t, nt, sh_cnt);
  __syncthreads();
  bin_flush(a, t, nt, sh_cnt);
}

__global__ void __launch_bounds__(PB_SORT_BIN_THREADS) k_msm_bin_scatter(SortArgs a) {
  __shared__ uint32_t sh_cnt[PB_SORT_MAX_BINS], sh_loc[PB_SORT_MAX_BINS], sh_base[PB_SORT_MAX_BINS], sh_scan[32];
  extern __shared__ SortEntry stage[];
  const uint32_t t = threadIdx.x, nt = blockDim.x;
  sort_zero(sh_cnt, a.nbins, t, nt);
  __syncthreads();
  bin_hist(a, blockIdx.x, blockIdx.y, t, nt, sh_cnt);
  __syncthreads();
  uint32_t total;
  const uint32_t run = block_exclusive_scan(scan_part_sum(sh_cnt, a.nbins, t, nt), sh_scan, &total);
  bin_reserve(a, t, nt, run, sh_cnt, sh_loc, sh_base);
  __syncthreads();
  bin_stage(a, blockIdx.x, blockIdx.y, t, nt, sh_cnt, sh_loc, stage);
  __syncthreads();
  bin_copy_out(a, t, nt, total, sh_loc, sh_base, stage);
}

__global__ void __launch_bounds__(PB_SORT_CHUNK_THREADS) k_msm_chunk_count(SortArgs a) {
  __shared__ uint32_t sh_cnt[PB_SORT_MAX_BIN_KEYS];
  const uint32_t t = threadIdx.x, nt = blockDim.x;
  SortChunk ch;
  for (uint32_t c = blockIdx.x; chunk_locate(a, c, ch); c += gridDim.x) {
    sort_zero(sh_cnt, ch.nkeys, t, nt);
    __syncthreads();
    chunk_hist(a, ch, t, nt, sh_cnt);
    __syncthreads();
    chunk_flush(a, ch, t, nt, sh_cnt);
    __syncthreads();
  }
}

__global__ void __launch_bounds__(PB_SORT_CHUNK_THREADS) k_msm_chunk_place(SortArgs a) {
  __shared__ uint32_t sh_cnt[PB_SORT_MAX_BIN_KEYS], sh_loc[PB_SORT_MAX_BIN_KEYS], sh_base[PB_SORT_MAX_BIN_KEYS],
      sh_scan[32];
  extern __shared__ uint32_t stage_vals[];
  const uint32_t t = threadIdx.x, nt = blockDim.x;
  SortChunk ch;
  for (uint32_t c = blockIdx.x; chunk_locate(a, c, ch); c += gridDim.x) {
    sort_zero(sh_cnt, ch.nkeys, t, nt);
    __syncthreads();
    chunk_hist(a, ch, t, nt, sh_cnt);
    __syncthreads();
    uint32_t total;
    const uint32_t run = block_exclusive_scan(scan_part_sum(sh_cnt, ch.nkeys, t, nt), sh_scan, &total);
    chunk_reserve(a, ch, t, nt, run, sh_cnt, sh_loc, sh_base);
    __syncthreads();
    chunk_stage(a, ch, t, nt, sh_cnt, sh_loc, stage_vals);
    __syncthreads();
    chunk_copy_out(a, ch, t, nt, sh_loc, sh_base, stage_vals);
    __syncthreads();
  }
}

#define PB_SCAN_TILE 2048

__global__ void __launch_bounds__(256) k_scan_tile_sums(const uint32_t* counts, uint32_t nb, uint32_t pad,
                                                        uint32_t* tile_sums, uint32_t* max_out) {
  __shared__ uint32_t sh[8];
  uint32_t base = blockIdx.x * PB_SCAN_TILE + threadIdx.x * 8;
  uint32_t s = 0, m = 0;
  for (int k = 0; k < 8; k++)
    if (base + k < nb) {
      uint32_t c = counts[base + k];
      m = max(m, c);
      s += (c + pad) & ~pad;
    }
  uint32_t total;
  block_exclusive_scan(s, sh, &total);
  if (threadIdx.x == 0) tile_sums[blockIdx.x] = total;
  if (max_out) {
    for (int d = 16; d > 0; d >>= 1) m = max(m, __shfl_xor_sync(0xffffffffu, m, d));
    if ((threadIdx.x & 31) == 0 && m) atomicMax(max_out, m);
  }
}

__global__ void __launch_bounds__(256) k_scan_tiles(uint32_t* tile_sums, uint32_t n_tiles, uint32_t* total_out) {
  __shared__ uint32_t sh[8];
  uint32_t per = (n_tiles + 255) / 256;
  uint32_t lo = threadIdx.x * per, hi = min(lo + per, n_tiles);
  uint32_t s = 0;
  for (uint32_t i = lo; i < hi; i++) s += tile_sums[i];
  uint32_t total;
  uint32_t run = block_exclusive_scan(s, sh, &total);
  for (uint32_t i = lo; i < hi; i++) {
    uint32_t c = tile_sums[i];
    tile_sums[i] = run;
    run += c;
  }
  if (threadIdx.x == 0) *total_out = total;
}

__global__ void __launch_bounds__(256) k_scan_apply(uint32_t* counts, uint32_t nb, uint32_t pad, const uint32_t* tile_sums,
                                                    uint32_t* offsets) {
  __shared__ uint32_t sh[8];
  uint32_t base = blockIdx.x * PB_SCAN_TILE + threadIdx.x * 8;
  uint32_t c[8];
  uint32_t s = 0;
  for (int k = 0; k < 8; k++) { c[k] = base + k < nb ? (counts[base + k] + pad) & ~pad : 0; s += c[k]; }
  uint32_t total;
  uint32_t run = tile_sums[blockIdx.x] + block_exclusive_scan(s, sh, &total);
  for (int k = 0; k < 8; k++) {
    if (base + k < nb) { offsets[base + k] = run; counts[base + k] = 0; }
    run += c[k];
  }
}

__global__ void __launch_bounds__(256) k_msm_chunk_map(SortArgs a) {
  __shared__ uint32_t sh[8];
  uint32_t total;
  const uint32_t run = block_exclusive_scan(chunk_map_sum(a, threadIdx.x), sh, &total);
  chunk_map_write(a, threadIdx.x, run, total);
}

__global__ void __launch_bounds__(128, 4) k_aff_round0(AffAcc a) {
  Fq pref[PB_AFF_BMAX];
  uint32_t desc[PB_AFF_BMAX];
  aff_round0_thread(a, (uint64_t)blockIdx.x * blockDim.x + threadIdx.x, pref, desc);
}
__global__ void __launch_bounds__(128, 4) k_aff_round(AffAcc a) {
  Fq pref[PB_AFF_BMAX];
  uint32_t desc[PB_AFF_BMAX];
  aff_round_thread(a, (uint64_t)blockIdx.x * blockDim.x + threadIdx.x, pref, desc);
}
__global__ void __launch_bounds__(256) k_aff_tail(AffAcc a, uint64_t s_bound) {
  Fq pref[PB_AFF_BMAX];
  uint32_t desc[PB_AFF_BMAX];
  const uint32_t maxc = *a.max_cnt;
  for (uint32_t r = PB_AFF_GRID_ROUNDS; r < 32 && maxc > (1u << r); r++) {
    a.r = r;
    const uint64_t T = aff_round_threads(s_bound, a.B, r);
    for (uint64_t t = threadIdx.x; t < T; t += blockDim.x) aff_round_thread(a, t, pref, desc);
    __syncthreads();
  }
}

#define PB_MSM_EMPTY 0xffffffffu

__device__ __forceinline__ uint32_t upper_bound_u32(const uint32_t* a, uint32_t n, uint32_t key) {
  uint32_t lo = 0, hi = n;
  while (lo < hi) {
    uint32_t mid = (lo + hi) >> 1;
    if (__ldg(a + mid) > key) hi = mid; else lo = mid + 1;
  }
  return lo;
}

__global__ void __launch_bounds__(128, 4) k_msm_seg_accumulate(const G1Affine* points, const uint32_t* offsets,
                                                            const uint32_t* sorted, uint32_t nb, uint32_t L,
                                                            G1XYZZ* buckets, G1XYZZ* slots, uint32_t* slot_bucket,
                                                            uint32_t* own_slot) {
  const uint32_t t = blockIdx.x * blockDim.x + threadIdx.x;
  const uint32_t M = offsets[nb];
  const uint64_t s64 = (uint64_t)t * L;
  if (s64 >= M) return;
  const uint32_t s = (uint32_t)s64;
  const uint32_t e = (uint32_t)min((uint64_t)M, s64 + L);
  uint32_t b = upper_bound_u32(offsets, nb + 1, s) - 1;
  uint32_t bstart = offsets[b], bend = offsets[b + 1];
  bool first = true;
  G1XYZZ acc = G1XYZZ::identity();
  for (uint32_t pos = s; pos <= e; pos++) {
    if (pos == bend || pos == e) {
      if (bstart >= s && bend <= e) {
        buckets[b] = acc;
      } else {
        uint32_t slot = first ? 2 * t : 2 * t + 1;
        slots[slot] = acc;
        slot_bucket[slot] = b;
        if (bstart >= s) own_slot[t] = slot;
      }
      if (pos == e) break;
      first = false;
      acc = G1XYZZ::identity();
      b++;
      while (offsets[b + 1] <= pos) b++;
      bstart = offsets[b];
      bend = offsets[b + 1];
    }
    uint32_t v = __ldg(sorted + pos);
    G1Affine p = ld_affine(points + (v & 0x7fffffffu));
    if (v >> 31) p.y = fp_neg(p.y);
    g1_add_mixed_uniform(acc, p);
  }
}

struct HeavyItem { uint32_t bucket, own_slot, t0, t1, piece_base, pieces; };
struct HeavyPiece { uint32_t item, index; };
#define PB_STITCH_PIECE 1024

__global__ void __launch_bounds__(128) k_msm_stitch(const uint32_t* offsets, uint32_t nb, uint32_t L,
                                                    uint32_t n_segments, const G1XYZZ* slots,
                                                    const uint32_t* slot_bucket, const uint32_t* own_slot,
                                                    G1XYZZ* buckets, HeavyItem* heavy, uint32_t* heavy_count,
                                                    HeavyPiece* pieces, uint32_t small_limit) {
  const uint32_t t = blockIdx.x * blockDim.x + threadIdx.x;
  if (t >= n_segments) return;
  const uint32_t os = own_slot[t];
  if (os == PB_MSM_EMPTY) return;
  const uint32_t b = slot_bucket[os];
  const uint32_t t1 = (offsets[b + 1] - 1) / L;
  if (t1 - t > small_limit) {
    uint32_t h = atomicAdd(heavy_count, 1u);
    HeavyItem it; it.bucket = b; it.own_slot = os; it.t0 = t; it.t1 = t1; it.piece_base = 0; it.pieces = 0;
    if (t1 - t > PB_STITCH_PIECE) {
      it.pieces = (t1 - t + PB_STITCH_PIECE - 1) / PB_STITCH_PIECE;
      it.piece_base = atomicAdd(heavy_count + 1, it.pieces);
      for (uint32_t p = 0; p < it.pieces; p++) { HeavyPiece hp; hp.item = h; hp.index = p; pieces[it.piece_base + p] = hp; }
    }
    heavy[h] = it;
    return;
  }
  G1XYZZ acc = slots[os];
  for (uint32_t k = t + 1; k <= t1; k++) {
    G1XYZZ piece = slots[2 * k];
    g1_add(acc, piece);
  }
  buckets[b] = acc;
}

__device__ __forceinline__ void block_sum_xyzz(G1XYZZ* sh, const G1XYZZ& mine) {
  sh[threadIdx.x] = mine;
  __syncthreads();
  for (uint32_t d = blockDim.x >> 1; d > 0; d >>= 1) {
    if (threadIdx.x < d) {
      G1XYZZ a = sh[threadIdx.x], c = sh[threadIdx.x + d];
      g1_add(a, c);
      sh[threadIdx.x] = a;
    }
    __syncthreads();
  }
}

__global__ void __launch_bounds__(128) k_msm_stitch_pieces(const G1XYZZ* slots, const HeavyItem* heavy,
                                                           const uint32_t* heavy_count, const HeavyPiece* pieces,
                                                           G1XYZZ* partial) {
  __shared__ G1XYZZ sh[128];
  const uint32_t count = heavy_count[1];
  for (uint32_t p = blockIdx.x; p < count; p += gridDim.x) {
    const HeavyPiece hp = pieces[p];
    const HeavyItem it = heavy[hp.item];
    const uint32_t lo = it.t0 + 1 + hp.index * PB_STITCH_PIECE;
    const uint32_t hi = min(lo + PB_STITCH_PIECE - 1, it.t1);
    G1XYZZ acc = G1XYZZ::identity();
    for (uint32_t k = lo + threadIdx.x; k <= hi; k += blockDim.x) {
      G1XYZZ piece = slots[2 * k];
      g1_add(acc, piece);
    }
    block_sum_xyzz(sh, acc);
    if (threadIdx.x == 0) partial[p] = sh[0];
    __syncthreads();
  }
}

__global__ void __launch_bounds__(128) k_msm_stitch_heavy(const G1XYZZ* slots, const HeavyItem* heavy,
                                                          const uint32_t* heavy_count, const G1XYZZ* partial,
                                                          G1XYZZ* buckets) {
  __shared__ G1XYZZ sh[128];
  const uint32_t count = *heavy_count;
  for (uint32_t h = blockIdx.x; h < count; h += gridDim.x) {
    HeavyItem it = heavy[h];
    G1XYZZ acc = G1XYZZ::identity();
    if (threadIdx.x == 0) acc = slots[it.own_slot];
    if (it.pieces) {
      for (uint32_t p = threadIdx.x; p < it.pieces; p += blockDim.x) {
        G1XYZZ piece = partial[it.piece_base + p];
        g1_add(acc, piece);
      }
    } else {
      for (uint32_t k = it.t0 + 1 + threadIdx.x; k <= it.t1; k += blockDim.x) {
        G1XYZZ piece = slots[2 * k];
        g1_add(acc, piece);
      }
    }
    block_sum_xyzz(sh, acc);
    if (threadIdx.x == 0) buckets[it.bucket] = sh[0];
    __syncthreads();
  }
}

__global__ void __launch_bounds__(128) k_reduce_level0(ReduceArgs a) {
  reduce_level0_thread(a, (uint64_t)blockIdx.x * blockDim.x + threadIdx.x);
}
__global__ void __launch_bounds__(PB_REDUCE_THREADS) k_reduce_block(BlockLevelArgs a) {
  __shared__ G1XYZZ sh[PB_REDUCE_THREADS];
  const uint32_t t = threadIdx.x, chunk = blockIdx.x, set = blockIdx.y;
  G1XYZZ s, x;
  blk_local(a, set, chunk, t, s, x);
  sh[t] = s;
  __syncthreads();
#pragma unroll 1
  for (uint32_t d = 1; d < PB_REDUCE_THREADS; d <<= 1) {
    const G1XYZZ v = blk_scan_step(sh, t, d);
    __syncthreads();
    sh[t] = v;
    __syncthreads();
  }
  const G1XYZZ suf = sh[t];
  const G1XYZZ y = blk_weight(a, t, x, suf);
  __syncthreads();
  sh[t] = y;
  __syncthreads();
#pragma unroll 1
  for (uint32_t d = PB_REDUCE_THREADS / 2; d > 0; d >>= 1) {
    blk_tree_step(sh, t, d);
    __syncthreads();
  }
  if (t == 0) {
    SR o;
    o.S = suf;
    o.R = sh[0];
    a.out[(uint64_t)set * gridDim.x + chunk] = o;
  }
}

__global__ void k_affine_to_mont(const G1Affine* in, G1Affine* out, uint64_t n) {
  uint64_t i = (uint64_t)blockIdx.x * blockDim.x + threadIdx.x;
  if (i >= n) return;
  G1Affine p = in[i];
  p.x = fp_to_mont(p.x);
  p.y = fp_to_mont(p.y);
  out[i] = p;
}

__global__ void k_affine_from_mont(const G1Affine* in, G1Affine* out, uint64_t n) {
  uint64_t i = (uint64_t)blockIdx.x * blockDim.x + threadIdx.x;
  if (i >= n) return;
  G1Affine p = in[i];
  p.x = fp_from_mont(p.x);
  p.y = fp_from_mont(p.y);
  out[i] = p;
}

__global__ void __launch_bounds__(128) k_window_step(const G1Affine* in, G1XYZZ* out, uint64_t n, uint32_t c) {
  uint64_t i = (uint64_t)blockIdx.x * blockDim.x + threadIdx.x;
  if (i >= n) return;
  G1Affine p = in[i];
  G1XYZZ a;
  g1_double_affine(a, p);
  for (uint32_t k = 1; k < c; k++) g1_double(a);
  out[i] = a;
}

void affine_to_mont(Context* ctx, const G1Affine* in, G1Affine* out, uint64_t n) {
  k_affine_to_mont<<<(unsigned)((n + 127) / 128), 128, 0, ctx->stream>>>(in, out, n);
  ctx->launches++;
  PB_CUDA(cudaGetLastError());
}

__global__ void __launch_bounds__(128) k_batch_to_affine(const G1XYZZ* in, G1Affine* out, uint64_t n) {
  const int CH = 16;
  uint64_t t = (uint64_t)blockIdx.x * blockDim.x + threadIdx.x;
  uint64_t i0 = t * CH;
  if (i0 >= n) return;
  int cnt = (int)min((uint64_t)CH, n - i0);
  Fq pref[CH];
  Fq run = Fq::one();
  for (int k = 0; k < cnt; k++) {
    pref[k] = run;
    run = fp_mul(run, in[i0 + k].ZZZ);
  }
  Fq inv = fp_inv_gcd(run);
  for (int k = cnt - 1; k >= 0; k--) {
    G1XYZZ a = in[i0 + k];
    Fq A = fp_mul(inv, pref[k]);
    inv = fp_mul(inv, a.ZZZ);
    Fq izz = fp_sqr(fp_mul(a.ZZ, A));
    G1Affine p;
    p.x = fp_mul(a.X, izz);
    p.y = fp_mul(a.Y, A);
    out[i0 + k] = p;
  }
}

struct Srs {
  uint64_t n = 0;
  DevBuf base;
  uint32_t c = 0, W = 0;
  DevBuf expanded;
};

static uint32_t windows_for(uint32_t c) { return (256 + c - 1) / c; }

uint32_t msm_default_window(uint64_t n, bool fixed_base) {
  int lg = 0;
  while (((uint64_t)1 << lg) < n) lg++;
  int c = fixed_base ? lg : lg - 4;
  int lo = 4, hi = fixed_base ? 21 : 16;
  if (const char* e = getenv(fixed_base ? "PB200_MSM_C_FIXED" : "PB200_MSM_C")) { c = atoi(e); }
  if (c < lo) c = lo;
  if (c > hi) c = hi;
  return (uint32_t)c;
}

static G1XYZZ host_mul_small(const G1XYZZ& p, uint32_t k) {
  G1XYZZ r = G1XYZZ::identity();
  for (int i = 31; i >= 0; i--) {
    g1_double(r);
    if ((k >> i) & 1) g1_add(r, p);
  }
  return r;
}

static void host_horner_to_affine(const std::vector<G1XYZZ>& ws, uint32_t c, uint8_t* out_xy, int* is_identity) {
  G1XYZZ r = G1XYZZ::identity();
  for (int w = (int)ws.size() - 1; w >= 0; w--) {
    if (w != (int)ws.size() - 1)
      for (uint32_t k = 0; k < c; k++) g1_double(r);
    g1_add(r, ws[w]);
  }
  G1Affine a;
  bool inf = g1_to_affine(r, a);
  *is_identity = inf ? 1 : 0;
  Fq x = fp_from_mont(a.x), y = fp_from_mont(a.y);
  memcpy(out_xy, x.v, 32);
  memcpy(out_xy + 32, y.v, 32);
}

static uint32_t env_u32(const char* name, uint32_t dflt) {
  const char* e = getenv(name);
  return e ? (uint32_t)atoi(e) : dflt;
}

static uint32_t pick_B(Context* ctx, uint64_t slots, uint32_t r) {
  static const uint32_t forced = env_u32("PB200_MSM_B", 0);
  const uint32_t cap = r == 0 ? 64 : PB_AFF_BMAX;
  if (forced) return std::min<uint32_t>(std::max<uint32_t>(r == 0 ? forced : 2 * forced, 2), cap);
  const uint64_t full = (uint64_t)ctx->sm_count * 256;
  for (uint32_t B = cap; B > 16; B >>= 1)
    if (slots / aff_round_span(B, r) >= 2 * full) return B;
  return 16;
}

void host_join_bucket_shards_strided(const SR* all, uint32_t world, uint32_t sets, G1XYZZ* out) {
  uint32_t log_g = 0;
  while ((1u << log_g) < world) log_g++;
  PB_CHECK((1u << log_g) == world, "strided bucket shards need a power-of-two rank count");
  for (uint32_t s = 0; s < sets; s++) {
    G1XYZZ run = G1XYZZ::identity(), weighted = G1XYZZ::identity(), plain = G1XYZZ::identity();
    for (uint32_t rho = 0; rho < world; rho++) {
      const SR& e = all[(size_t)rho * sets + s];
      g1_add(plain, e.R);
      if (rho + 1 < world) {
        g1_add(run, e.S);
        g1_add(weighted, run);
      }
    }
    for (uint32_t k = 0; k < log_g; k++) g1_double(plain);
    weighted.Y = fp_neg(weighted.Y);
    g1_add(plain, weighted);
    out[s] = plain;
  }
}

void host_join_bucket_shards(const SR* all, uint32_t world, uint32_t sets, uint32_t nloc, G1XYZZ* out) {
  uint32_t log_nloc = 0;
  while ((1u << log_nloc) < nloc) log_nloc++;
  PB_CHECK((1u << log_nloc) == nloc, "bucket shards must be a power of two wide");
  for (uint32_t s = 0; s < sets; s++) {
    G1XYZZ run = G1XYZZ::identity(), weighted = G1XYZZ::identity(), plain = G1XYZZ::identity();
    for (uint32_t rho = world; rho-- > 0;) {
      const SR& e = all[(size_t)rho * sets + s];
      g1_add(plain, e.R);
      if (rho >= 1) {
        g1_add(run, e.S);
        g1_add(weighted, run);
      }
    }
    for (uint32_t k = 0; k < log_nloc; k++) g1_double(weighted);
    g1_add(plain, weighted);
    out[s] = plain;
  }
}

void msm_run_batch(Context* ctx, const G1Affine* points, uint64_t n, const Fr* const* scalars, uint32_t batch,
                   bool scalars_mont, uint32_t c, bool fixed_base, uint64_t point_stride, uint32_t bucket_lo,
                   uint32_t bucket_hi, uint8_t* out_xy , int* is_identity ,
                   G1XYZZ* raw_out , Comm* comm = nullptr) {
  PB_CHECK(n > 0, "empty MSM");
  PB_CHECK(batch >= 1 && batch <= 4 && (fixed_base || batch == 1), "bad MSM batch");
  MsmGeom g;
  g.c = c;
  g.W = windows_for(c);
  g.half = 1u << (c - 1);
  g.fixed_base = fixed_base ? 1 : 0;
  g.point_stride = fixed_base ? point_stride : 0;
  g.batch = batch;
  g.own_log = 0;
  g.own_rank = 0;
  if (comm && comm_world(comm) > 1) {
    PB_CHECK((g.half >> comm_log_world(comm)) >= 1, "more ranks than buckets");
    static const bool contiguous = getenv("PB200_SHARD_CONTIGUOUS") != nullptr;
    if (contiguous) {
      const uint32_t per = g.half >> comm_log_world(comm);
      bucket_lo = per * (uint32_t)comm_rank(comm);
      bucket_hi = bucket_lo + per;
    } else {
      g.own_log = (uint32_t)comm_log_world(comm);
      g.own_rank = (uint32_t)comm_rank(comm);
      bucket_lo = 0;
      bucket_hi = g.half >> g.own_log;
    }
  } else {
    comm = nullptr;
  }
  if (bucket_hi > g.half) bucket_hi = g.half;
  PB_CHECK(bucket_lo < bucket_hi, "empty MSM bucket range");
  g.lo = bucket_lo;
  g.nloc = bucket_hi - bucket_lo;
  g.sets = fixed_base ? batch : g.W;
  g.nb = g.sets * g.nloc;
  PB_CHECK((fixed_base ? (uint64_t)g.W * point_stride : n) < (1ull << 31), "MSM too large for 31-bit point ids");
  ScalarBatch sb;
  for (uint32_t k = 0; k < 4; k++) sb.p[k] = k < batch ? scalars[k] : nullptr;

  static const bool use_xyzz = [] { const char* e = getenv("PB200_MSM_ACC"); return !(e && !strcmp(e, "affine")); }();
  const uint32_t pad = use_xyzz ? 0 : 1;
  DevBuf& sorted = ctx->scratch[2];
  DevBuf& counts = ctx->scratch[3];
  DevBuf& offsets = ctx->scratch[4];
  DevBuf& lvl_a = ctx->scratch[6];
  DevBuf& lvl_b = ctx->scratch[7];
  const uint64_t entries = n * g.W * batch;
  const uint64_t positions = entries + (pad ? g.nb : 0);
  PB_CHECK(positions < (1ull << 30), "MSM too large (n * windows * batch must stay below 2^30)");
  sorted.ensure(positions * 4);
  counts.ensure((size_t)g.nb * 4 + 16);
  offsets.ensure((size_t)(g.nb + 1) * 4);
  uint32_t* max_cnt = counts.as<uint32_t>() + g.nb;
  const uint32_t n_tiles = (g.nb + PB_SCAN_TILE - 1) / PB_SCAN_TILE;
  PB_CHECK(n_tiles <= 8192, "too many buckets for the scan");
  ctx->msm_aff[1].ensure((size_t)8192 * 4);
  uint32_t* tile_sums = ctx->msm_aff[1].as<uint32_t>();

  const uint32_t lb = sort_default_lb(g.nb);
  PB_CHECK((1u << lb) <= PB_SORT_MAX_BIN_KEYS, "too many buckets for the sort");
  DevBuf& binned = ctx->scratch[8];
  DevBuf& bin_tab = ctx->scratch[9];
  binned.ensure(entries * sizeof(SortEntry));
  bin_tab.ensure((size_t)3 * (PB_SORT_MAX_BINS + 1) * 4);
  SortArgs sa;
  sa.sb = sb;
  sa.n = n;
  sa.from_mont = scalars_mont ? 1 : 0;
  sa.g = g;
  sa.lb = lb;
  sa.nbins = ((g.nb - 1) >> lb) + 1;
  sa.T = PB_SORT_CHUNK;
  uint32_t* bin_cnt = bin_tab.as<uint32_t>();
  uint32_t* bin_off = bin_cnt + PB_SORT_MAX_BINS + 1;
  sa.bin_cnt = bin_cnt;
  sa.bin_off = bin_off;
  sa.binned = binned.as<SortEntry>();
  sa.chunk_first = bin_off + PB_SORT_MAX_BINS + 1;
  sa.counts = counts.as<uint32_t>();
  sa.offsets = offsets.as<uint32_t>();
  sa.sorted = sorted.as<uint32_t>();
  sa.spb = PB_SORT_BIN_STAGE / g.W;
  const dim3 bin_grid((unsigned)((n + sa.spb - 1) / sa.spb), batch);
  const uint64_t chunk_bound = entries / PB_SORT_CHUNK + sa.nbins;
  const uint32_t count_grid = (uint32_t)std::min<uint64_t>((uint64_t)ctx->sm_count * 4, chunk_bound);
  const uint32_t place_grid = (uint32_t)std::min<uint64_t>((uint64_t)ctx->sm_count * 2, chunk_bound);
  const size_t bin_stage_bytes = PB_SORT_BIN_STAGE * sizeof(SortEntry), chunk_stage_bytes = PB_SORT_CHUNK * 4;
  PB_CUDA(cudaFuncSetAttribute(k_msm_bin_scatter, cudaFuncAttributeMaxDynamicSharedMemorySize, (int)bin_stage_bytes));
  PB_CUDA(cudaFuncSetAttribute(k_msm_chunk_place, cudaFuncAttributeMaxDynamicSharedMemorySize, (int)chunk_stage_bytes));

  cudaStream_t st = ctx->stream;
  ctx->time_begin(2);
  PB_CUDA(cudaMemsetAsync(counts.p, 0, (size_t)g.nb * 4 + 16, st));
  PB_CUDA(cudaMemsetAsync(bin_cnt, 0, (size_t)sa.nbins * 4, st));
  if (pad) PB_CUDA(cudaMemsetAsync(sorted.p, 0xff, positions * 4, st));
  k_msm_bin_count<<<bin_grid, PB_SORT_BIN_THREADS, 0, st>>>(sa);
  k_scan_tile_sums<<<1, 256, 0, st>>>(bin_cnt, sa.nbins, 0, tile_sums, nullptr);
  k_scan_tiles<<<1, 256, 0, st>>>(tile_sums, 1, bin_off + sa.nbins);
  k_scan_apply<<<1, 256, 0, st>>>(bin_cnt, sa.nbins, 0, tile_sums, bin_off);
  k_msm_bin_scatter<<<bin_grid, PB_SORT_BIN_THREADS, bin_stage_bytes, st>>>(sa);
  k_msm_chunk_map<<<1, 256, 0, st>>>(sa);
  k_msm_chunk_count<<<count_grid, PB_SORT_CHUNK_THREADS, 0, st>>>(sa);
  k_scan_tile_sums<<<n_tiles, 256, 0, st>>>(counts.as<uint32_t>(), g.nb, pad, tile_sums, max_cnt);
  k_scan_tiles<<<1, 256, 0, st>>>(tile_sums, n_tiles, offsets.as<uint32_t>() + g.nb);
  k_scan_apply<<<n_tiles, 256, 0, st>>>(counts.as<uint32_t>(), g.nb, pad, tile_sums, offsets.as<uint32_t>());
  k_msm_chunk_place<<<place_grid, PB_SORT_CHUNK_THREADS, chunk_stage_bytes, st>>>(sa);
  ctx->time_end(2);
  ctx->launches += 11;

  ReduceArgs ra;
  ra.pts = nullptr; ra.off = offsets.as<uint32_t>(); ra.cnt = counts.as<uint32_t>(); ra.xb = nullptr;
  if (!use_xyzz) {
    const uint64_t s_bound = positions / 2;
    DevBuf& pts = ctx->msm_aff[0];
    pts.ensure(s_bound * sizeof(G1Affine));
    AffAcc a;
    a.table = points;
    a.sorted = sorted.as<uint32_t>();
    a.pts = pts.as<G1Affine>();
    a.off = offsets.as<uint32_t>();
    a.cnt = counts.as<uint32_t>();
    a.max_cnt = max_cnt;
    a.nbl = g.nb;
    uint64_t cap = fixed_base ? n * g.W : n;
    uint32_t max_rounds = 1;
    while (max_rounds < 32 && (1ull << max_rounds) < cap) max_rounds++;
    ctx->time_begin(0);
    for (uint32_t r = 0; r < std::min<uint32_t>(max_rounds, PB_AFF_GRID_ROUNDS); r++) {
      a.r = r;
      a.B = pick_B(ctx, s_bound, r);
      const uint64_t threads = aff_round_threads(s_bound, a.B, r);
      if (r == 0) k_aff_round0<<<(unsigned)((threads + 127) / 128), 128, 0, st>>>(a);
      else k_aff_round<<<(unsigned)((threads + 127) / 128), 128, 0, st>>>(a);
      ctx->launches++;
    }
    if (max_rounds > PB_AFF_GRID_ROUNDS) {
      a.B = 32;
      k_aff_tail<<<1, 256, 0, st>>>(a, s_bound);
      ctx->launches++;
    }
    ctx->time_end(0);
    ra.pts = pts.as<G1Affine>();
  } else {
    DevBuf& buckets = ctx->scratch[5];
    DevBuf& seg = ctx->scratch[1];
    buckets.ensure((size_t)g.nb * sizeof(G1XYZZ));
    static const uint32_t seg_env = env_u32("PB200_MSM_SEG", 0);
    uint32_t L = 32;
    if (seg_env) {
      L = seg_env;
    } else {
      const uint64_t expected = entries / (g.half / g.nloc);
      while (L > 4 && expected / L < (uint64_t)ctx->sm_count * 512) L >>= 1;
      while (L < 32 && (entries / L) * (2 * sizeof(G1XYZZ) + 12 + sizeof(HeavyItem)) > (1ull << 30)) L <<= 1;
    }
    PB_CHECK(L >= 1 && L <= 4096, "bad PB200_MSM_SEG");
    const uint32_t n_seg = (uint32_t)((entries + L - 1) / L);
    const uint32_t max_pieces = 2 * (n_seg / PB_STITCH_PIECE) + 16;
    seg.ensure((size_t)n_seg * 2 * sizeof(G1XYZZ) + (size_t)n_seg * 3 * 4 + (size_t)n_seg * sizeof(HeavyItem) + 16 +
               (size_t)max_pieces * (sizeof(HeavyPiece) + sizeof(G1XYZZ)));
    G1XYZZ* slots = seg.as<G1XYZZ>();
    G1XYZZ* piece_partial = slots + (size_t)n_seg * 2;
    uint32_t* slot_bucket = reinterpret_cast<uint32_t*>(piece_partial + max_pieces);
    uint32_t* own_slot = slot_bucket + (size_t)n_seg * 2;
    uint32_t* heavy_count = own_slot + n_seg;
    HeavyItem* heavy = reinterpret_cast<HeavyItem*>(heavy_count + 4);
    HeavyPiece* pieces = reinterpret_cast<HeavyPiece*>(heavy + n_seg);
    PB_CUDA(cudaMemsetAsync(buckets.p, 0, (size_t)g.nb * sizeof(G1XYZZ), st));
    PB_CUDA(cudaMemsetAsync(own_slot, 0xff, (size_t)n_seg * 4, st));
    PB_CUDA(cudaMemsetAsync(heavy_count, 0, 16, st));
    ctx->time_begin(0);
    k_msm_seg_accumulate<<<(n_seg + 127) / 128, 128, 0, st>>>(points, offsets.as<uint32_t>(), sorted.as<uint32_t>(),
                                                             g.nb, L, buckets.as<G1XYZZ>(), slots, slot_bucket, own_slot);
    ctx->time_end(0);
    k_msm_stitch<<<(n_seg + 127) / 128, 128, 0, st>>>(offsets.as<uint32_t>(), g.nb, L, n_seg, slots, slot_bucket,
                                                     own_slot, buckets.as<G1XYZZ>(), heavy, heavy_count, pieces, 16);
    k_msm_stitch_pieces<<<std::min<uint32_t>(max_pieces, 592), 128, 0, st>>>(slots, heavy, heavy_count, pieces, piece_partial);
    k_msm_stitch_heavy<<<296, 128, 0, st>>>(slots, heavy, heavy_count, piece_partial, buckets.as<G1XYZZ>());
    ctx->launches += 4;
    ra.xb = buckets.as<G1XYZZ>();
  }

  static const uint32_t g0_env = env_u32("PB200_MSM_G", 0);
  uint32_t log_g0 = 4;
  if (g0_env) {
    log_g0 = 1;
    while ((2u << log_g0) <= g0_env && log_g0 < 10) log_g0++;
  } else {
    while (log_g0 > 2 && (g.nb >> log_g0) < (uint32_t)ctx->sm_count * 256) log_g0--;
  }
  ctx->time_begin(3);
  ra.sets = g.sets;
  ra.m = g.nloc;
  ra.g = 1u << log_g0;
  {
    const uint64_t groups = (uint64_t)g.sets * reduce_groups(ra.m, ra.g);
    lvl_a.ensure(groups * sizeof(SR));
    lvl_b.ensure((groups / 16 + g.sets) * sizeof(SR));
    ra.out = lvl_a.as<SR>();
    k_reduce_level0<<<(unsigned)((groups + 127) / 128), 128, 0, st>>>(ra);
    ctx->launches++;
  }
  uint32_t m = reduce_groups(ra.m, ra.g), log_G = log_g0;
  SR* cur = lvl_a.as<SR>();
  SR* nxt = lvl_b.as<SR>();
  const uint32_t m_stop = comm ? 1 : 8;
  while (m > m_stop) {
    BlockLevelArgs ba;
    ba.in = cur; ba.out = nxt; ba.sets = g.sets; ba.m = m; ba.log_G = log_G;
    k_reduce_block<<<dim3(reduce_chunks(m), g.sets), PB_REDUCE_THREADS, 0, st>>>(ba);
    ctx->launches++;
    m = reduce_chunks(m);
    log_G += 9;
    std::swap(cur, nxt);
  }
  ctx->time_end(3);
  PB_CUDA(cudaGetLastError());
  std::vector<G1XYZZ> ws(g.sets);
  if (comm) {
    const uint32_t world = (uint32_t)comm_world(comm);
    DevBuf& gath = ctx->msm_aff[2];
    const size_t per_rank = (size_t)g.sets * m;
    gath.ensure((size_t)world * per_rank * sizeof(SR));
    SR* all = gath.as<SR>();
    PB_CUDA(cudaMemcpyAsync(all + (size_t)comm_rank(comm) * per_rank, cur, per_rank * sizeof(SR), cudaMemcpyDeviceToDevice, st));
    comm_allgather_inplace(comm, all, per_rank * sizeof(SR), st);
    std::vector<SR> raw((size_t)world * per_rank), fin((size_t)world * g.sets);
    PB_CUDA(cudaMemcpyAsync(raw.data(), all, raw.size() * sizeof(SR), cudaMemcpyDeviceToHost, st));
    PB_CUDA(cudaStreamSynchronize(st));
    for (uint32_t rho = 0; rho < world; rho++)
      for (uint32_t s = 0; s < g.sets; s++)
        fin[(size_t)rho * g.sets + s] = reduce_fold_final(raw.data() + (size_t)rho * per_rank + (size_t)s * m, m, log_G);
    if (g.own_log) host_join_bucket_shards_strided(fin.data(), world, g.sets, ws.data());
    else host_join_bucket_shards(fin.data(), world, g.sets, g.nloc, ws.data());
  } else {
    std::vector<SR> raw((size_t)g.sets * m), fin(g.sets);
    PB_CUDA(cudaMemcpyAsync(raw.data(), cur, raw.size() * sizeof(SR), cudaMemcpyDeviceToHost, st));
    PB_CUDA(cudaStreamSynchronize(st));
    for (uint32_t s = 0; s < g.sets; s++) fin[s] = reduce_fold_final(raw.data() + (size_t)s * m, m, log_G);
    for (uint32_t s = 0; s < g.sets; s++) {
      ws[s] = fin[s].R;
      if (g.lo) {
        G1XYZZ m_lo = host_mul_small(fin[s].S, g.lo);
        g1_add(ws[s], m_lo);
      }
    }
  }
  if (raw_out) {
    if (fixed_base) {
      for (uint32_t k = 0; k < batch; k++) raw_out[k] = ws[k];
    } else {
      G1XYZZ r = G1XYZZ::identity();
      for (int w = (int)g.W - 1; w >= 0; w--) {
        if (w != (int)g.W - 1) for (uint32_t k = 0; k < c; k++) g1_double(r);
        g1_add(r, ws[w]);
      }
      raw_out[0] = r;
    }
  } else if (fixed_base) {
    for (uint32_t k = 0; k < batch; k++) {
      std::vector<G1XYZZ> one(1, ws[k]);
      host_horner_to_affine(one, c, out_xy + 64 * k, is_identity + k);
    }
  } else {
    host_horner_to_affine(ws, c, out_xy, is_identity);
  }
}

void msm_run(Context* ctx, const G1Affine* points, uint64_t n, const Fr* scalars, bool scalars_mont, uint32_t c,
             bool fixed_base, uint64_t point_stride, uint8_t* out_xy, int* is_identity) {
  msm_run_batch(ctx, points, n, &scalars, 1, scalars_mont, c, fixed_base, point_stride, 0, 0xffffffffu, out_xy,
                is_identity, nullptr);
}

static void srs_finish(Context* ctx, Srs* srs, int precompute);

Srs* srs_create(Context* ctx, const uint8_t* h_points, uint64_t n, int precompute) {
  auto srs = std::make_unique<Srs>();
  srs->n = n;
  srs->base.alloc(n * sizeof(G1Affine));
  DevBuf raw(n * sizeof(G1Affine));
  PB_CUDA(cudaMemcpyAsync(raw.p, h_points, n * sizeof(G1Affine), cudaMemcpyHostToDevice, ctx->stream));
  k_affine_to_mont<<<(unsigned)((n + 127) / 128), 128, 0, ctx->stream>>>(raw.as<G1Affine>(), srs->base.as<G1Affine>(), n);
  ctx->launches++;
  PB_CUDA(cudaStreamSynchronize(ctx->stream));
  srs_finish(ctx, srs.get(), precompute);
  return srs.release();
}

static void srs_finish(Context* ctx, Srs* srs, int precompute) {
  const uint64_t n = srs->n;
  if (precompute) {
    uint32_t c = msm_default_window(n, true);
    uint32_t W = windows_for(c);
    srs->c = c;
    srs->W = W;
    srs->expanded.alloc((size_t)W * n * sizeof(G1Affine));
    G1Affine* ex = srs->expanded.as<G1Affine>();
    PB_CUDA(cudaMemcpyAsync(ex, srs->base.p, n * sizeof(G1Affine), cudaMemcpyDeviceToDevice, ctx->stream));
    DevBuf tmp(n * sizeof(G1XYZZ));
    for (uint32_t w = 1; w < W; w++) {
      k_window_step<<<(unsigned)((n + 127) / 128), 128, 0, ctx->stream>>>(ex + (uint64_t)(w - 1) * n, tmp.as<G1XYZZ>(), n, c);
      uint64_t threads = (n + 15) / 16;
      k_batch_to_affine<<<(unsigned)((threads + 127) / 128), 128, 0, ctx->stream>>>(tmp.as<G1XYZZ>(), ex + (uint64_t)w * n, n);
      ctx->launches += 2;
    }
    PB_CUDA(cudaStreamSynchronize(ctx->stream));
  }
  PB_CUDA(cudaGetLastError());
}

void srs_destroy(Srs* s) { delete s; }


__global__ void __launch_bounds__(128) k_fb_table(G1XYZZ* out) {
  uint32_t t = blockIdx.x * blockDim.x + threadIdx.x;
  if (t >= 32 * 255) return;
  uint32_t w = t / 255, d = t % 255 + 1;
  G1Affine g;
  g.x = Fq::one();
  g.y = fp_add(Fq::one(), Fq::one());
  G1XYZZ gx = g1_from_affine(g);
  G1XYZZ r = G1XYZZ::identity();
  for (int i = 7; i >= 0; i--) {
    g1_double(r);
    if ((d >> i) & 1) g1_add(r, gx);
  }
  for (uint32_t k = 0; k < 8 * w; k++) g1_double(r);
  out[t] = r;
}

__global__ void __launch_bounds__(128) k_fb_mul(const G1Affine* table, const Fr* scalars_mont, uint64_t n, G1XYZZ* out) {
  uint64_t i = (uint64_t)blockIdx.x * blockDim.x + threadIdx.x;
  if (i >= n) return;
  Fr s = fp_from_mont(scalars_mont[i]);
  G1XYZZ acc = G1XYZZ::identity();
  for (uint32_t w = 0; w < 32; w++) {
    uint32_t d = (s.v[w >> 2] >> (8 * (w & 3))) & 0xff;
    if (d) {
      G1Affine p = ld_affine(table + w * 255 + (d - 1));
      g1_add_mixed(acc, p);
    }
  }
  out[i] = acc;
}

void launch_powers(Context* ctx, Fr* out, uint64_t n, const Fr& base, const Fr& scale);
static void srs_finish(Context* ctx, Srs* srs, int precompute);

void ntt_run(Context* ctx, const Fr* in, Fr* out, int log_n, bool inverse, uint64_t n_in, const Fr* in_scale,
             const Fr* out_scale);

static Srs* srs_from_tau(Context* ctx, const Fr& tau_canonical, uint64_t n, int precompute, bool lagrange) {
  auto srs = std::make_unique<Srs>();
  srs->n = n;
  srs->base.alloc(n * sizeof(G1Affine));
  cudaStream_t st = ctx->stream;
  DevBuf tab_x(32 * 255 * sizeof(G1XYZZ)), tab(32 * 255 * sizeof(G1Affine));
  k_fb_table<<<(32 * 255 + 127) / 128, 128, 0, st>>>(tab_x.as<G1XYZZ>());
  k_batch_to_affine<<<((32 * 255 + 15) / 16 + 127) / 128, 128, 0, st>>>(tab_x.as<G1XYZZ>(), tab.as<G1Affine>(), 32 * 255);
  DevBuf pw(n * 32), pts(n * sizeof(G1XYZZ)), lag;
  launch_powers(ctx, pw.as<Fr>(), n, fp_to_mont(tau_canonical), Fr::one());
  const Fr* scalars = pw.as<Fr>();
  if (lagrange) {
    int log_n = 0;
    while (((uint64_t)1 << log_n) < n) log_n++;
    PB_CHECK(((uint64_t)1 << log_n) == n, "the Lagrange basis needs a power-of-two domain");
    lag.alloc(n * 32);
    ntt_run(ctx, pw.as<Fr>(), lag.as<Fr>(), log_n, true, n, nullptr, nullptr);
    scalars = lag.as<Fr>();
  }
  k_fb_mul<<<(unsigned)((n + 127) / 128), 128, 0, st>>>(tab.as<G1Affine>(), scalars, n, pts.as<G1XYZZ>());
  uint64_t threads = (n + 15) / 16;
  k_batch_to_affine<<<(unsigned)((threads + 127) / 128), 128, 0, st>>>(pts.as<G1XYZZ>(), srs->base.as<G1Affine>(), n);
  ctx->launches += 4;
  PB_CUDA(cudaStreamSynchronize(st));
  srs_finish(ctx, srs.get(), precompute);
  return srs.release();
}
Srs* srs_generate(Context* ctx, const Fr& tau_canonical, uint64_t n, int precompute) {
  return srs_from_tau(ctx, tau_canonical, n, precompute, false);
}
Srs* srs_generate_lagrange(Context* ctx, const Fr& tau_canonical, uint64_t n, int precompute) {
  return srs_from_tau(ctx, tau_canonical, n, precompute, true);
}

void srs_export(Context* ctx, Srs* srs, uint8_t* h_points, uint64_t first, uint64_t count) {
  PB_CHECK(first + count <= srs->n, "SRS export out of range");
  DevBuf tmp(count * sizeof(G1Affine));
  k_affine_from_mont<<<(unsigned)((count + 127) / 128), 128, 0, ctx->stream>>>(srs->base.as<G1Affine>() + first,
                                                                          tmp.as<G1Affine>(), count);
  ctx->launches++;
  PB_CUDA(cudaMemcpyAsync(h_points, tmp.p, count * sizeof(G1Affine), cudaMemcpyDeviceToHost, ctx->stream));
  PB_CUDA(cudaStreamSynchronize(ctx->stream));
}

void srs_msm(Context* ctx, Srs* srs, const Fr* d_scalars, uint64_t m, bool scalars_mont, uint8_t* out_xy, int* is_identity) {
  PB_CHECK(m <= srs->n, "Not enough powers in setup");
  if (srs->expanded.p) {
    msm_run(ctx, srs->expanded.as<G1Affine>(), m, d_scalars, scalars_mont, srs->c, true, srs->n, out_xy, is_identity);
  } else {
    msm_run(ctx, srs->base.as<G1Affine>(), m, d_scalars, scalars_mont, msm_default_window(m, false), false, 0, out_xy,
            is_identity);
  }
}

void srs_msm_batch(Context* ctx, Srs* srs, const Fr* const* d_scalars, uint32_t batch, uint64_t m, bool scalars_mont,
                   uint8_t* out_xy, int* is_identity) {
  PB_CHECK(m <= srs->n, "Not enough powers in setup");
  if (srs->expanded.p && batch > 1) {
    msm_run_batch(ctx, srs->expanded.as<G1Affine>(), m, d_scalars, batch, scalars_mont, srs->c, true, srs->n, 0,
                  0xffffffffu, out_xy, is_identity, nullptr);
  } else {
    for (uint32_t k = 0; k < batch; k++) srs_msm(ctx, srs, d_scalars[k], m, scalars_mont, out_xy + 64 * k, is_identity + k);
  }
}

void srs_msm_batch_partial(Context* ctx, Srs* srs, const Fr* const* d_scalars, uint32_t batch, uint64_t first,
                           uint64_t count, uint32_t bucket_lo, uint32_t bucket_hi, bool scalars_mont, G1XYZZ* out) {
  PB_CHECK(first + count <= srs->n, "Not enough powers in setup");
  PB_CHECK(srs->expanded.p, "sharded commitments need the fixed-base table (precompute)");
  const Fr* sh[4] = {nullptr, nullptr, nullptr, nullptr};
  for (uint32_t k = 0; k < batch; k++) sh[k] = d_scalars[k] + first;
  if (count == 0 || bucket_lo >= bucket_hi) {
    for (uint32_t k = 0; k < batch; k++) out[k] = G1XYZZ::identity();
    return;
  }
  msm_run_batch(ctx, srs->expanded.as<G1Affine>() + first, count, sh, batch, scalars_mont, srs->c, true, srs->n,
                bucket_lo, bucket_hi, nullptr, nullptr, out);
}
uint32_t srs_bucket_count(Srs* s) { return s->c ? 1u << (s->c - 1) : 0; }

void srs_msm_batch_sharded(Context* ctx, Srs* srs, const Fr* const* d_scalars, uint32_t batch, uint64_t m,
                           bool scalars_mont, uint8_t* out_xy, int* is_identity) {
  PB_CHECK(m <= srs->n, "Not enough powers in setup");
  PB_CHECK(srs->expanded.p, "sharded commitments need the fixed-base table (precompute)");
  PB_CHECK(ctx->comm, "sharded commitments need a communicator on the context (pb200_comm_init)");
  msm_run_batch(ctx, srs->expanded.as<G1Affine>(), m, d_scalars, batch, scalars_mont, srs->c, true, srs->n, 0,
                0xffffffffu, out_xy, is_identity, nullptr, ctx->comm);
}

void g1_combine_partials_host(const G1XYZZ* parts, uint32_t count, uint8_t* out_xy, int* is_identity) {
  std::vector<G1XYZZ> ws(1, G1XYZZ::identity());
  for (uint32_t k = 0; k < count; k++) g1_add(ws[0], parts[k]);
  host_horner_to_affine(ws, 1, out_xy, is_identity);
}

uint64_t srs_size(Srs* s) { return s->n; }
const G1Affine* srs_base(Srs* s) { return s->base.as<G1Affine>(); }

}
```

### plonkathon_b200/csrc/msm_digits.cuh

```cuda
#pragma once
#include "field.cuh"

namespace pb200 {

struct MsmGeom {
  uint32_t c, W;
  uint32_t half;
  uint32_t fixed_base;
  uint64_t point_stride;
  uint32_t batch;
  uint32_t lo, nloc;
  uint32_t own_log, own_rank;
  uint32_t sets;
  uint32_t nb;
};

PB_HD uint32_t msm_bucket_key(const MsmGeom& g, uint32_t k, uint32_t w, uint32_t d) {
  uint32_t j;
  if (g.own_log) {
    if (((d - 1) & ((1u << g.own_log) - 1)) != g.own_rank) return 0xffffffffu;
    j = (d - 1) >> g.own_log;
  } else {
    j = d - 1 - g.lo;
    if (j >= g.nloc) return 0xffffffffu;
  }
  return (g.fixed_base ? k : w) * g.nloc + j;
}

struct ScalarBatch { const Fr* p[4]; };

struct DigitWalk {
  Fr s;
  uint32_t carry;
  PB_HD DigitWalk(const Fr* scalars, uint64_t i, int from_mont) : carry(0) {
    s = scalars[i];
    if (from_mont) s = fp_from_mont(s);
  }
  PB_HD uint32_t next(uint32_t w, const MsmGeom& g, uint32_t& neg) {
    uint32_t bit = w * g.c;
    uint32_t limb = bit >> 5, off = bit & 31;
    uint64_t two = limb < 8 ? s.v[limb] : 0;
    if (limb + 1 < 8) two |= (uint64_t)s.v[limb + 1] << 32;
    uint32_t raw = (uint32_t)(two >> off) & ((1u << g.c) - 1);
    uint32_t d = raw + carry;
    neg = 0;
    if (d > g.half) { d = (1u << g.c) - d; neg = 1; carry = 1; } else carry = 0;
    return d;
  }
};


}
```

### plonkathon_b200/csrc/msm_sort.cuh

```cuda
#pragma once
#include "msm_digits.cuh"

namespace pb200 {

#define PB_SORT_MAX_BINS 2048
#define PB_SORT_MAX_BIN_KEYS 2048
#define PB_SORT_BIN_THREADS 512
#define PB_SORT_BIN_STAGE 8192
#define PB_SORT_CHUNK_THREADS 512
#define PB_SORT_CHUNK 16384
static_assert(PB_SORT_MAX_BINS <= 256 * 8, "k_msm_chunk_map and the bin scan take one block of 256 x 8 bins");

struct alignas(8) SortEntry {
  uint32_t key, val;
};

struct SortArgs {
  ScalarBatch sb;
  uint64_t n;
  int from_mont;
  MsmGeom g;
  uint32_t spb;
  uint32_t lb;
  uint32_t nbins;
  uint32_t T;
  uint32_t* bin_cnt;
  const uint32_t* bin_off;
  SortEntry* binned;
  uint32_t* chunk_first;
  uint32_t* counts;
  const uint32_t* offsets;
  uint32_t* sorted;
};

PB_HD uint32_t sort_default_lb(uint32_t nb) {
  uint32_t lb = 0;
  while (((nb - 1) >> lb) >= PB_SORT_MAX_BINS) lb++;
  return lb;
}

PB_HD uint32_t sort_add(uint32_t* p, uint32_t v) {
#if defined(__CUDA_ARCH__)
  return atomicAdd(p, v);
#else
  const uint32_t o = *p;
  *p = o + v;
  return o;
#endif
}

PB_HD void sort_zero(uint32_t* sh, uint32_t len, uint32_t t, uint32_t nt) {
  for (uint32_t b = t; b < len; b += nt) sh[b] = 0;
}

PB_HD uint32_t scan_part_sum(const uint32_t* sh, uint32_t len, uint32_t t, uint32_t nt) {
  const uint32_t per = (len + nt - 1) / nt;
  uint32_t s = 0;
  for (uint32_t b = t * per; b < t * per + per && b < len; b++) s += sh[b];
  return s;
}

template <class F>
PB_HD void sort_walk(const SortArgs& a, uint32_t bx, uint32_t k, uint32_t t, uint32_t nt, F f) {
  const uint64_t end = (uint64_t)(bx + 1) * a.spb < a.n ? (uint64_t)(bx + 1) * a.spb : a.n;
  for (uint64_t i = (uint64_t)bx * a.spb + t; i < end; i += nt) {
    DigitWalk dw(a.sb.p[k], i, a.from_mont);
    for (uint32_t w = 0; w < a.g.W; w++) {
      uint32_t neg, d = dw.next(w, a.g, neg);
      if (!d) continue;
      const uint32_t key = msm_bucket_key(a.g, k, w, d);
      if (key != 0xffffffffu) f(key, (uint32_t)((uint64_t)w * a.g.point_stride + i) | (neg << 31));
    }
  }
}

PB_HD void bin_hist(const SortArgs& a, uint32_t bx, uint32_t k, uint32_t t, uint32_t nt, uint32_t* sh_cnt) {
  sort_walk(a, bx, k, t, nt, [&](uint32_t key, uint32_t) { sort_add(&sh_cnt[key >> a.lb], 1u); });
}

PB_HD void bin_flush(const SortArgs& a, uint32_t t, uint32_t nt, const uint32_t* sh_cnt) {
  for (uint32_t b = t; b < a.nbins; b += nt)
    if (sh_cnt[b]) sort_add(&a.bin_cnt[b], sh_cnt[b]);
}

PB_HD void bin_reserve(const SortArgs& a, uint32_t t, uint32_t nt, uint32_t run, uint32_t* sh_cnt, uint32_t* sh_loc,
                       uint32_t* sh_base) {
  const uint32_t per = (a.nbins + nt - 1) / nt;
  for (uint32_t b = t * per; b < t * per + per && b < a.nbins; b++) {
    const uint32_t c = sh_cnt[b];
    sh_loc[b] = run;
    run += c;
    if (c) sh_base[b] = a.bin_off[b] + sort_add(&a.bin_cnt[b], c);
    sh_cnt[b] = 0;
  }
}

PB_HD void bin_stage(const SortArgs& a, uint32_t bx, uint32_t k, uint32_t t, uint32_t nt, uint32_t* sh_cnt,
                     const uint32_t* sh_loc, SortEntry* stage) {
  sort_walk(a, bx, k, t, nt, [&](uint32_t key, uint32_t val) {
    const uint32_t b = key >> a.lb;
    SortEntry e;
    e.key = key;
    e.val = val;
    stage[sh_loc[b] + sort_add(&sh_cnt[b], 1u)] = e;
  });
}

PB_HD void bin_copy_out(const SortArgs& a, uint32_t t, uint32_t nt, uint32_t total, const uint32_t* sh_loc,
                        const uint32_t* sh_base, const SortEntry* stage) {
  for (uint32_t p = t; p < total; p += nt) {
    const SortEntry e = stage[p];
    const uint32_t b = e.key >> a.lb;
    a.binned[sh_base[b] + p - sh_loc[b]] = e;
  }
}

PB_HD uint32_t chunk_map_sum(const SortArgs& a, uint32_t t) {
  uint32_t s = 0;
  for (uint32_t b = 8 * t; b < 8 * t + 8 && b < a.nbins; b++) s += (a.bin_cnt[b] + a.T - 1) / a.T;
  return s;
}
PB_HD void chunk_map_write(const SortArgs& a, uint32_t t, uint32_t run, uint32_t total) {
  for (uint32_t b = 8 * t; b < 8 * t + 8 && b < a.nbins; b++) {
    a.chunk_first[b] = run;
    run += (a.bin_cnt[b] + a.T - 1) / a.T;
  }
  if (t == 0) a.chunk_first[a.nbins] = total;
}

struct SortChunk {
  uint32_t lo, hi;
  uint32_t key0, nkeys;
};

PB_HD bool chunk_locate(const SortArgs& a, uint32_t c, SortChunk& ch) {
  if (c >= a.chunk_first[a.nbins]) return false;
  uint32_t l = 0, h = a.nbins;
  while (l < h) {
    const uint32_t m = (l + h) >> 1;
    if (a.chunk_first[m] > c) h = m; else l = m + 1;
  }
  const uint32_t b = l - 1;
  ch.lo = a.bin_off[b] + (c - a.chunk_first[b]) * a.T;
  ch.hi = a.bin_off[b + 1] - ch.lo > a.T ? ch.lo + a.T : a.bin_off[b + 1];
  ch.key0 = b << a.lb;
  ch.nkeys = a.g.nb - ch.key0 < (1u << a.lb) ? a.g.nb - ch.key0 : 1u << a.lb;
  return true;
}

PB_HD void chunk_hist(const SortArgs& a, const SortChunk& ch, uint32_t t, uint32_t nt, uint32_t* sh_cnt) {
  for (uint32_t i = ch.lo + t; i < ch.hi; i += nt) sort_add(&sh_cnt[a.binned[i].key - ch.key0], 1u);
}

PB_HD void chunk_flush(const SortArgs& a, const SortChunk& ch, uint32_t t, uint32_t nt, const uint32_t* sh_cnt) {
  for (uint32_t l = t; l < ch.nkeys; l += nt)
    if (sh_cnt[l]) sort_add(&a.counts[ch.key0 + l], sh_cnt[l]);
}

PB_HD void chunk_reserve(const SortArgs& a, const SortChunk& ch, uint32_t t, uint32_t nt, uint32_t run,
                         uint32_t* sh_cnt, uint32_t* sh_loc, uint32_t* sh_base) {
  const uint32_t per = (ch.nkeys + nt - 1) / nt;
  for (uint32_t l = t * per; l < t * per + per && l < ch.nkeys; l++) {
    const uint32_t c = sh_cnt[l];
    sh_loc[l] = run;
    run += c;
    if (c) sh_base[l] = a.offsets[ch.key0 + l] + sort_add(&a.counts[ch.key0 + l], c);
    sh_cnt[l] = 0;
  }
}

PB_HD void chunk_stage(const SortArgs& a, const SortChunk& ch, uint32_t t, uint32_t nt, uint32_t* sh_cnt,
                       const uint32_t* sh_loc, uint32_t* stage) {
  for (uint32_t i = ch.lo + t; i < ch.hi; i += nt) {
    const SortEntry e = a.binned[i];
    const uint32_t l = e.key - ch.key0;
    stage[sh_loc[l] + sort_add(&sh_cnt[l], 1u)] = e.val;
  }
}

PB_HD void chunk_copy_out(const SortArgs& a, const SortChunk& ch, uint32_t t, uint32_t nt, const uint32_t* sh_loc,
                          const uint32_t* sh_base, const uint32_t* stage) {
  for (uint32_t p = t; p < ch.hi - ch.lo; p += nt) {
    uint32_t lo = 0, hi = ch.nkeys;
    while (lo < hi) {
      const uint32_t m = (lo + hi) >> 1;
      if (sh_loc[m] > p) hi = m; else lo = m + 1;
    }
    a.sorted[sh_base[lo - 1] + p - sh_loc[lo - 1]] = stage[p];
  }
}

}
```

Measured before the change: 20.68.

## Restructure MSM bucket sort with bin-local placement and cached scalars in scatter

Reworks the MSM counting sort. Scalars are cached in shared memory during the scatter histogram so digits are not recomputed from global memory. Bins small enough for one block are now fully sorted and placed by a new per-bin kernel, which also computes offsets and the max count, replacing the global scan kernels in the unpadded path. The chunk map is folded into a single bin-scan kernel, and thread counts and stage sizes are raised. A batched commit API is also added. This cuts kernel launches and global passes, at the cost of more shared memory per block and more intricate code paths.

```diff
diff --git a/include/plonk_b200.h b/include/plonk_b200.h
--- a/include/plonk_b200.h
+++ b/include/plonk_b200.h
@@ -110,6 +110,8 @@
 int pb200_srs_commit_partial(pb200_ctx* ctx, pb200_srs* srs, const void* d_coeffs, uint64_t first, uint64_t count,
                              uint32_t bucket_lo, uint32_t bucket_hi, int coeffs_montgomery, uint8_t* h_xyzz128);
 int pb200_srs_bucket_count(pb200_srs* srs, uint32_t* out);
+int pb200_srs_commit_coeffs_batch(pb200_ctx* ctx, pb200_srs* srs, const void* const* h_d_coeffs, unsigned batch,
+                                  uint64_t m, int coeffs_montgomery, uint8_t* h_out_xy, int* is_identity);
 int pb200_g1_combine_partials_host(const uint8_t* h_xyzz, unsigned count, uint8_t* h_out_xy, int* is_identity);
 int pb200_g1_join_bucket_shards_host(const uint8_t* h_sr, unsigned world, unsigned sets, uint32_t nloc, uint8_t* h_out_xy,
                                      int* is_identity);
diff --git a/plonkathon_b200/_lib.py b/plonkathon_b200/_lib.py
--- a/plonkathon_b200/_lib.py
+++ b/plonkathon_b200/_lib.py
@@ -47,6 +47,7 @@
         "pb200_prover_create_sharded": (I, [V, V, U, V, P(V)]),
         "pb200_srs_commit_partial": (I, [V, V, V, U64, U64, U, U, I, V]),
         "pb200_srs_bucket_count": (I, [V, P(U)]),
+        "pb200_srs_commit_coeffs_batch": (I, [V, V, V, U, U64, I, V, P(I)]),
         "pb200_g1_join_bucket_shards_host": (I, [V, U, U, U, V, P(I)]),
         "pb200_fr_coset_extend": (I, [V, V, V, U, V]),
         "pb200_fr_coset_extend_host": (I, [V, V, V, U, V]),
diff --git a/plonkathon_b200/csrc/capi.cu b/plonkathon_b200/csrc/capi.cu
--- a/plonkathon_b200/csrc/capi.cu
+++ b/plonkathon_b200/csrc/capi.cu
@@ -587,6 +587,15 @@
   memcpy(h_xyzz128, &part, sizeof(part));
   PB_API_END
 }
+int pb200_srs_commit_coeffs_batch(pb200_ctx* ctx, pb200_srs* srs, const void* const* h_d_coeffs, unsigned batch,
+                                  uint64_t m, int coeffs_montgomery, uint8_t* h_out_xy, int* is_identity) {
+  PB_API_BEGIN PB_ON_CTX(C(ctx));
+  PB_CHECK(batch >= 1 && batch <= 4, "batch must be 1..4");
+  const Fr* sc[4];
+  for (unsigned k = 0; k < batch; k++) sc[k] = (const Fr*)h_d_coeffs[k];
+  srs_msm_batch(C(ctx), reinterpret_cast<Srs*>(srs), sc, batch, m, coeffs_montgomery != 0, h_out_xy, is_identity);
+  PB_API_END
+}
 int pb200_srs_bucket_count(pb200_srs* srs, uint32_t* out) {
   PB_API_BEGIN
   *out = srs_bucket_count(reinterpret_cast<Srs*>(srs));
diff --git a/plonkathon_b200/csrc/host_selftest.cpp b/plonkathon_b200/csrc/host_selftest.cpp
--- a/plonkathon_b200/csrc/host_selftest.cpp
+++ b/plonkathon_b200/csrc/host_selftest.cpp
@@ -259,6 +259,7 @@
   a.n = n;
   a.from_mont = 0;
   a.g = g;
+  a.pad = pad;
   a.lb = lb;
   a.nbins = nbins;
   a.T = T;
@@ -271,8 +272,10 @@
   a.sorted = nullptr;
   a.spb = spb;
   std::vector<uint32_t> sh_cnt(std::max(nbins, 1u << lb)), sh_loc(sh_cnt.size()), sh_base(sh_cnt.size()), runs;
-  std::vector<SortEntry> bin_stage_buf((size_t)spb * g.W);
-  std::vector<uint32_t> chunk_stage_buf(T);
+  std::vector<SortEntry> stage_buf(std::max<size_t>((size_t)spb * g.W, T));
+  std::vector<Fr> sh_sc(spb);
+  std::vector<uint32_t> stage_vals(T);
+  uint32_t sh_max = 0;
   auto block_scan = [&](uint32_t len, uint32_t nt) {
     runs.assign(nt, 0);
     uint32_t run = 0;
@@ -286,25 +289,29 @@
       for (uint32_t t = 0; t < bin_nt; t++) bin_hist(a, bx, k, t, bin_nt, sh_cnt.data());
       for (uint32_t t = 0; t < bin_nt; t++) bin_flush(a, t, bin_nt, sh_cnt.data());
     }
-  host_scan(bin_cnt.data(), nbins, 0, bin_off.data(), nullptr);
+  {
+    std::vector<uint32_t> se(bin_nt), sc_(bin_nt);
+    for (uint32_t t = 0; t < bin_nt; t++) bin_scan_sums(a, t, bin_nt, se[t], sc_[t]);
+    uint32_t te = 0, tc = 0;
+    for (uint32_t t = 0; t < bin_nt; t++) {
+      const uint32_t e = se[t], c = sc_[t];
+      se[t] = te;
+      sc_[t] = tc;
+      te += e;
+      tc += c;
+    }
+    for (uint32_t t = 0; t < bin_nt; t++) bin_scan_write(a, t, bin_nt, se[t], sc_[t], te, tc);
+  }
   for (uint32_t k = batch; k-- > 0;)
     for (uint32_t bx = bin_blocks; bx-- > 0;) {
       for (uint32_t t = 0; t < bin_nt; t++) sort_zero(sh_cnt.data(), nbins, t, bin_nt);
-      for (uint32_t t = 0; t < bin_nt; t++) bin_hist(a, bx, k, t, bin_nt, sh_cnt.data());
+      for (uint32_t t = 0; t < bin_nt; t++) scatter_hist(a, bx, k, t, bin_nt, sh_cnt.data(), sh_sc.data());
       const uint32_t total = block_scan(nbins, bin_nt);
+      for (uint32_t t = 0; t < bin_nt; t++) scatter_reserve(a, t, bin_nt, runs[t], sh_cnt.data(), sh_base.data());
       for (uint32_t t = 0; t < bin_nt; t++)
-        bin_reserve(a, t, bin_nt, runs[t], sh_cnt.data(), sh_loc.data(), sh_base.data());
-      for (uint32_t t = 0; t < bin_nt; t++) bin_stage(a, bx, k, t, bin_nt, sh_cnt.data(), sh_loc.data(), bin_stage_buf.data());
-      for (uint32_t t = 0; t < bin_nt; t++)
-        bin_copy_out(a, t, bin_nt, total, sh_loc.data(), sh_base.data(), bin_stage_buf.data());
-    }
-  {
-    std::vector<uint32_t> sums(256);
-    for (uint32_t t = 0; t < 256; t++) sums[t] = chunk_map_sum(a, t);
-    uint32_t run = 0;
-    for (uint32_t t = 0; t < 256; t++) { const uint32_t s = sums[t]; sums[t] = run; run += s; }
-    for (uint32_t t = 0; t < 256; t++) chunk_map_write(a, t, sums[t], run);
-  }
+        scatter_stage(a, bx, k, t, bin_nt, sh_cnt.data(), sh_sc.data(), stage_buf.data());
+      for (uint32_t t = 0; t < bin_nt; t++) scatter_copy_out(a, t, bin_nt, total, sh_base.data(), stage_buf.data());
+    }
   const uint32_t grid = 3;
   SortChunk ch;
   for (uint32_t bx = 0; bx < grid; bx++)
@@ -313,9 +320,26 @@
       for (uint32_t t = 0; t < chunk_nt; t++) chunk_hist(a, ch, t, chunk_nt, sh_cnt.data());
       for (uint32_t t = 0; t < chunk_nt; t++) chunk_flush(a, ch, t, chunk_nt, sh_cnt.data());
     }
-  host_scan(counts.data(), g.nb, pad, off.data(), &counts[g.nb]);
-  sorted.assign(off[g.nb] + 2, PB_MSM_PAD);
-  a.sorted = sorted.data();
+  if (pad) {
+    host_scan(counts.data(), g.nb, pad, off.data(), &counts[g.nb]);
+    sorted.assign(off[g.nb] + 2, PB_MSM_PAD);
+    a.sorted = sorted.data();
+  } else {
+    sorted.assign(off[g.nb] + 2, PB_MSM_PAD);
+    a.sorted = sorted.data();
+    for (uint32_t b = nbins; b-- > 0;) {
+      const SortBin s = sort_bin(a, b);
+      for (uint32_t t = 0; t < chunk_nt; t++) sort_zero(sh_cnt.data(), s.nkeys, t, chunk_nt);
+      sh_max = 0;
+      for (uint32_t t = 0; t < chunk_nt; t++) place_hist(a, s, t, chunk_nt, sh_cnt.data(), stage_buf.data());
+      const uint32_t total = block_scan(s.nkeys, chunk_nt);
+      if (total != s.hi - s.lo) abort();
+      for (uint32_t t = 0; t < chunk_nt; t++) place_reserve(a, s, t, chunk_nt, runs[t], sh_cnt.data(), &sh_max);
+      for (uint32_t t = 0; t < chunk_nt; t++)
+        place_stage(a, s, t, chunk_nt, sh_cnt.data(), &sh_max, stage_buf.data(), stage_vals.data());
+      for (uint32_t t = 0; t < chunk_nt; t++) place_copy_out(a, s, t, chunk_nt, stage_vals.data());
+    }
+  }
   for (uint32_t bx = grid; bx-- > 0;)
     for (uint32_t c = bx; chunk_locate(a, c, ch); c += grid) {
       for (uint32_t t = 0; t < chunk_nt; t++) sort_zero(sh_cnt.data(), ch.nkeys, t, chunk_nt);
@@ -323,9 +347,9 @@
       const uint32_t total = block_scan(ch.nkeys, chunk_nt);
       for (uint32_t t = 0; t < chunk_nt; t++)
         chunk_reserve(a, ch, t, chunk_nt, runs[t], sh_cnt.data(), sh_loc.data(), sh_base.data());
-      for (uint32_t t = 0; t < chunk_nt; t++) chunk_stage(a, ch, t, chunk_nt, sh_cnt.data(), sh_loc.data(), chunk_stage_buf.data());
+      for (uint32_t t = 0; t < chunk_nt; t++) chunk_stage(a, ch, t, chunk_nt, sh_cnt.data(), sh_loc.data(), stage_vals.data());
       for (uint32_t t = 0; t < chunk_nt; t++)
-        chunk_copy_out(a, ch, t, chunk_nt, sh_loc.data(), sh_base.data(), chunk_stage_buf.data());
+        chunk_copy_out(a, ch, t, chunk_nt, sh_loc.data(), sh_base.data(), stage_vals.data());
       if (total != ch.hi - ch.lo) abort();
     }
 }
@@ -340,7 +364,8 @@
   if (!msm_geom(n, batch, c, fixed_base, lo, hi, g)) return -1;
   if (lb == 0xffffffffu) lb = sort_default_lb(g.nb);
   if (((g.nb - 1) >> lb) >= PB_SORT_MAX_BINS || (1u << lb) > PB_SORT_MAX_BIN_KEYS) return -1;
-  if (!spb) spb = PB_SORT_BIN_STAGE / g.W;
+  if (T >= (1u << (32 - PB_SORT_KEY_BITS))) return -1;
+  if (!spb) spb = sort_default_spb(g.W);
   std::vector<Fr> sc((size_t)batch * n);
   for (size_t i = 0; i < sc.size(); i++) sc[i] = ld<Fr>(scalars + 8 * i);
   std::vector<uint32_t> counts, off, sorted;
@@ -374,7 +399,7 @@
   std::vector<Fr> sc((size_t)batch * n);
   for (size_t i = 0; i < sc.size(); i++) sc[i] = ld<Fr>(scalars + 8 * i);
   std::vector<uint32_t> counts, off, sorted;
-  host_msm_sort(g, sc, n, 1, sort_default_lb(g.nb), PB_SORT_CHUNK, PB_SORT_BIN_STAGE / g.W, PB_SORT_BIN_THREADS,
+  host_msm_sort(g, sc, n, 1, sort_default_lb(g.nb), PB_SORT_CHUNK, sort_default_spb(g.W), PB_SORT_BIN_THREADS,
                 PB_SORT_CHUNK_THREADS, counts, off, sorted);
   const uint32_t maxc = counts[g.nb];
   const uint64_t positions = (uint64_t)n * g.W * batch + g.nb, s_bound = positions / 2;
diff --git a/plonkathon_b200/csrc/msm.cu b/plonkathon_b200/csrc/msm.cu
--- a/plonkathon_b200/csrc/msm.cu
+++ b/plonkathon_b200/csrc/msm.cu
@@ -54,21 +54,52 @@
   bin_flush(a, t, nt, sh_cnt);
 }
 
-__global__ void __launch_bounds__(PB_SORT_BIN_THREADS) k_msm_bin_scatter(SortArgs a) {
-  __shared__ uint32_t sh_cnt[PB_SORT_MAX_BINS], sh_loc[PB_SORT_MAX_BINS], sh_base[PB_SORT_MAX_BINS], sh_scan[32];
-  extern __shared__ SortEntry stage[];
+__global__ void __launch_bounds__(PB_SORT_SCAN_THREADS) k_msm_bin_scan(SortArgs a) {
+  __shared__ uint32_t sh[32];
+  const uint32_t t = threadIdx.x, nt = blockDim.x;
+  uint32_t e, c, total_e, total_c;
+  bin_scan_sums(a, t, nt, e, c);
+  const uint32_t run_e = block_exclusive_scan(e, sh, &total_e);
+  const uint32_t run_c = block_exclusive_scan(c, sh, &total_c);
+  bin_scan_write(a, t, nt, run_e, run_c, total_e, total_c);
+}
+
+__global__ void __launch_bounds__(PB_SORT_SCATTER_THREADS) k_msm_bin_scatter(SortArgs a) {
+  __shared__ uint32_t sh_cnt[PB_SORT_MAX_BINS], sh_delta[PB_SORT_MAX_BINS], sh_scan[32];
+  extern __shared__ __align__(16) Fr sh_sc[];
+  SortEntry* stage = reinterpret_cast<SortEntry*>(sh_sc + a.spb);
   const uint32_t t = threadIdx.x, nt = blockDim.x;
   sort_zero(sh_cnt, a.nbins, t, nt);
   __syncthreads();
-  bin_hist(a, blockIdx.x, blockIdx.y, t, nt, sh_cnt);
+  scatter_hist(a, blockIdx.x, blockIdx.y, t, nt, sh_cnt, sh_sc);
   __syncthreads();
   uint32_t total;
   const uint32_t run = block_exclusive_scan(scan_part_sum(sh_cnt, a.nbins, t, nt), sh_scan, &total);
-  bin_reserve(a, t, nt, run, sh_cnt, sh_loc, sh_base);
-  __syncthreads();
-  bin_stage(a, blockIdx.x, blockIdx.y, t, nt, sh_cnt, sh_loc, stage);
-  __syncthreads();
-  bin_copy_out(a, t, nt, total, sh_loc, sh_base, stage);
+  scatter_reserve(a, t, nt, run, sh_cnt, sh_delta);
+  __syncthreads();
+  scatter_stage(a, blockIdx.x, blockIdx.y, t, nt, sh_cnt, sh_sc, stage);
+  __syncthreads();
+  scatter_copy_out(a, t, nt, total, sh_delta, stage);
+}
+
+__global__ void __launch_bounds__(PB_SORT_PLACE_THREADS) k_msm_bin_place(SortArgs a) {
+  __shared__ uint32_t sh_cnt[PB_SORT_MAX_BIN_KEYS], sh_scan[32], sh_max;
+  extern __shared__ SortEntry stage[];
+  uint32_t* stage_vals = reinterpret_cast<uint32_t*>(stage + a.T);
+  const uint32_t t = threadIdx.x, nt = blockDim.x;
+  const SortBin s = sort_bin(a, blockIdx.x);
+  sort_zero(sh_cnt, s.nkeys, t, nt);
+  if (t == 0) sh_max = 0;
+  __syncthreads();
+  place_hist(a, s, t, nt, sh_cnt, stage);
+  __syncthreads();
+  uint32_t total;
+  const uint32_t run = block_exclusive_scan(scan_part_sum(sh_cnt, s.nkeys, t, nt), sh_scan, &total);
+  place_reserve(a, s, t, nt, run, sh_cnt, &sh_max);
+  __syncthreads();
+  place_stage(a, s, t, nt, sh_cnt, &sh_max, stage, stage_vals);
+  __syncthreads();
+  place_copy_out(a, s, t, nt, stage_vals);
 }
 
 __global__ void __launch_bounds__(PB_SORT_CHUNK_THREADS) k_msm_chunk_count(SortArgs a) {
@@ -158,13 +189,6 @@
     if (base + k < nb) { offsets[base + k] = run; counts[base + k] = 0; }
     run += c[k];
   }
-}
-
-__global__ void __launch_bounds__(256) k_msm_chunk_map(SortArgs a) {
-  __shared__ uint32_t sh[8];
-  uint32_t total;
-  const uint32_t run = block_exclusive_scan(chunk_map_sum(a, threadIdx.x), sh, &total);
-  chunk_map_write(a, threadIdx.x, run, total);
 }
 
 __global__ void __launch_bounds__(128, 4) k_aff_round0(AffAcc a) {
@@ -598,6 +622,7 @@
   sa.n = n;
   sa.from_mont = scalars_mont ? 1 : 0;
   sa.g = g;
+  sa.pad = pad;
   sa.lb = lb;
   sa.nbins = ((g.nb - 1) >> lb) + 1;
   sa.T = PB_SORT_CHUNK;
@@ -610,14 +635,17 @@
   sa.counts = counts.as<uint32_t>();
   sa.offsets = offsets.as<uint32_t>();
   sa.sorted = sorted.as<uint32_t>();
-  sa.spb = PB_SORT_BIN_STAGE / g.W;
+  sa.spb = sort_default_spb(g.W);
   const dim3 bin_grid((unsigned)((n + sa.spb - 1) / sa.spb), batch);
   const uint64_t chunk_bound = entries / PB_SORT_CHUNK + sa.nbins;
   const uint32_t count_grid = (uint32_t)std::min<uint64_t>((uint64_t)ctx->sm_count * 4, chunk_bound);
   const uint32_t place_grid = (uint32_t)std::min<uint64_t>((uint64_t)ctx->sm_count * 2, chunk_bound);
-  const size_t bin_stage_bytes = PB_SORT_BIN_STAGE * sizeof(SortEntry), chunk_stage_bytes = PB_SORT_CHUNK * 4;
-  PB_CUDA(cudaFuncSetAttribute(k_msm_bin_scatter, cudaFuncAttributeMaxDynamicSharedMemorySize, (int)bin_stage_bytes));
-  PB_CUDA(cudaFuncSetAttribute(k_msm_chunk_place, cudaFuncAttributeMaxDynamicSharedMemorySize, (int)chunk_stage_bytes));
+  const size_t scatter_smem = (size_t)sa.spb * (g.W * sizeof(SortEntry) + sizeof(Fr));
+  const size_t place_smem = (size_t)PB_SORT_CHUNK * (sizeof(SortEntry) + 4), chunk_smem = (size_t)PB_SORT_CHUNK * 4;
+  PB_CHECK(scatter_smem <= 180 * 1024, "too few windows for the bin scatter's shared memory");
+  PB_CUDA(cudaFuncSetAttribute(k_msm_bin_scatter, cudaFuncAttributeMaxDynamicSharedMemorySize, (int)scatter_smem));
+  PB_CUDA(cudaFuncSetAttribute(k_msm_bin_place, cudaFuncAttributeMaxDynamicSharedMemorySize, (int)place_smem));
+  PB_CUDA(cudaFuncSetAttribute(k_msm_chunk_place, cudaFuncAttributeMaxDynamicSharedMemorySize, (int)chunk_smem));
 
   cudaStream_t st = ctx->stream;
   ctx->time_begin(2);
@@ -625,18 +653,19 @@
   PB_CUDA(cudaMemsetAsync(bin_cnt, 0, (size_t)sa.nbins * 4, st));
   if (pad) PB_CUDA(cudaMemsetAsync(sorted.p, 0xff, positions * 4, st));
   k_msm_bin_count<<<bin_grid, PB_SORT_BIN_THREADS, 0, st>>>(sa);
-  k_scan_tile_sums<<<1, 256, 0, st>>>(bin_cnt, sa.nbins, 0, tile_sums, nullptr);
-  k_scan_tiles<<<1, 256, 0, st>>>(tile_sums, 1, bin_off + sa.nbins);
-  k_scan_apply<<<1, 256, 0, st>>>(bin_cnt, sa.nbins, 0, tile_sums, bin_off);
-  k_msm_bin_scatter<<<bin_grid, PB_SORT_BIN_THREADS, bin_stage_bytes, st>>>(sa);
-  k_msm_chunk_map<<<1, 256, 0, st>>>(sa);
+  k_msm_bin_scan<<<1, PB_SORT_SCAN_THREADS, 0, st>>>(sa);
+  k_msm_bin_scatter<<<bin_grid, PB_SORT_SCATTER_THREADS, scatter_smem, st>>>(sa);
   k_msm_chunk_count<<<count_grid, PB_SORT_CHUNK_THREADS, 0, st>>>(sa);
-  k_scan_tile_sums<<<n_tiles, 256, 0, st>>>(counts.as<uint32_t>(), g.nb, pad, tile_sums, max_cnt);
-  k_scan_tiles<<<1, 256, 0, st>>>(tile_sums, n_tiles, offsets.as<uint32_t>() + g.nb);
-  k_scan_apply<<<n_tiles, 256, 0, st>>>(counts.as<uint32_t>(), g.nb, pad, tile_sums, offsets.as<uint32_t>());
-  k_msm_chunk_place<<<place_grid, PB_SORT_CHUNK_THREADS, chunk_stage_bytes, st>>>(sa);
+  if (pad) {
+    k_scan_tile_sums<<<n_tiles, 256, 0, st>>>(counts.as<uint32_t>(), g.nb, pad, tile_sums, max_cnt);
+    k_scan_tiles<<<1, 256, 0, st>>>(tile_sums, n_tiles, offsets.as<uint32_t>() + g.nb);
+    k_scan_apply<<<n_tiles, 256, 0, st>>>(counts.as<uint32_t>(), g.nb, pad, tile_sums, offsets.as<uint32_t>());
+  } else {
+    k_msm_bin_place<<<sa.nbins, PB_SORT_PLACE_THREADS, place_smem, st>>>(sa);
+  }
+  k_msm_chunk_place<<<place_grid, PB_SORT_CHUNK_THREADS, chunk_smem, st>>>(sa);
   ctx->time_end(2);
-  ctx->launches += 11;
+  ctx->launches += pad ? 8 : 6;
 
   ReduceArgs ra;
   ra.pts = nullptr; ra.off = offsets.as<uint32_t>(); ra.cnt = counts.as<uint32_t>(); ra.xb = nullptr;
diff --git a/plonkathon_b200/csrc/msm_digits.cuh b/plonkathon_b200/csrc/msm_digits.cuh
--- a/plonkathon_b200/csrc/msm_digits.cuh
+++ b/plonkathon_b200/csrc/msm_digits.cuh
@@ -36,6 +36,7 @@
     s = scalars[i];
     if (from_mont) s = fp_from_mont(s);
   }
+  PB_HD explicit DigitWalk(const Fr& canonical) : s(canonical), carry(0) {}
   PB_HD uint32_t next(uint32_t w, const MsmGeom& g, uint32_t& neg) {
     uint32_t bit = w * g.c;
     uint32_t limb = bit >> 5, off = bit & 31;
diff --git a/plonkathon_b200/csrc/msm_sort.cuh b/plonkathon_b200/csrc/msm_sort.cuh
--- a/plonkathon_b200/csrc/msm_sort.cuh
+++ b/plonkathon_b200/csrc/msm_sort.cuh
@@ -3,13 +3,18 @@
 
 namespace pb200 {
 
-#define PB_SORT_MAX_BINS 2048
+#define PB_SORT_MAX_BINS 4096
 #define PB_SORT_MAX_BIN_KEYS 2048
 #define PB_SORT_BIN_THREADS 512
-#define PB_SORT_BIN_STAGE 8192
+#define PB_SORT_SCATTER_THREADS 1024
+#define PB_SORT_BIN_STAGE 16384
+#define PB_SORT_SCAN_THREADS 1024
+#define PB_SORT_PLACE_THREADS 1024
 #define PB_SORT_CHUNK_THREADS 512
 #define PB_SORT_CHUNK 16384
-static_assert(PB_SORT_MAX_BINS <= 256 * 8, "k_msm_chunk_map and the bin scan take one block of 256 x 8 bins");
+#define PB_SORT_KEY_BITS 11
+static_assert(PB_SORT_MAX_BIN_KEYS <= (1u << PB_SORT_KEY_BITS), "local keys must fit PB_SORT_KEY_BITS");
+static_assert(PB_SORT_CHUNK < (1u << (32 - PB_SORT_KEY_BITS)), "ranks must fit the rest of the word");
 
 struct alignas(8) SortEntry {
   uint32_t key, val;
@@ -20,16 +25,17 @@
   uint64_t n;
   int from_mont;
   MsmGeom g;
+  uint32_t pad;
   uint32_t spb;
   uint32_t lb;
   uint32_t nbins;
   uint32_t T;
   uint32_t* bin_cnt;
-  const uint32_t* bin_off;
+  uint32_t* bin_off;
   SortEntry* binned;
   uint32_t* chunk_first;
   uint32_t* counts;
-  const uint32_t* offsets;
+  uint32_t* offsets;
   uint32_t* sorted;
 };
 
@@ -37,6 +43,11 @@
   uint32_t lb = 0;
   while (((nb - 1) >> lb) >= PB_SORT_MAX_BINS) lb++;
   return lb;
+}
+
+PB_HD uint32_t sort_default_spb(uint32_t W) {
+  const uint32_t s = PB_SORT_BIN_STAGE / W;
+  return s >= PB_SORT_SCATTER_THREADS ? s / PB_SORT_SCATTER_THREADS * PB_SORT_SCATTER_THREADS : s;
 }
 
 PB_HD uint32_t sort_add(uint32_t* p, uint32_t v) {
@@ -48,6 +59,13 @@
   return o;
 #endif
 }
+PB_HD void sort_max(uint32_t* p, uint32_t v) {
+#if defined(__CUDA_ARCH__)
+  atomicMax(p, v);
+#else
+  if (v > *p) *p = v;
+#endif
+}
 
 PB_HD void sort_zero(uint32_t* sh, uint32_t len, uint32_t t, uint32_t nt) {
   for (uint32_t b = t; b < len; b += nt) sh[b] = 0;
@@ -61,21 +79,30 @@
 }
 
 template <class F>
-PB_HD void sort_walk(const SortArgs& a, uint32_t bx, uint32_t k, uint32_t t, uint32_t nt, F f) {
-  const uint64_t end = (uint64_t)(bx + 1) * a.spb < a.n ? (uint64_t)(bx + 1) * a.spb : a.n;
-  for (uint64_t i = (uint64_t)bx * a.spb + t; i < end; i += nt) {
-    DigitWalk dw(a.sb.p[k], i, a.from_mont);
-    for (uint32_t w = 0; w < a.g.W; w++) {
-      uint32_t neg, d = dw.next(w, a.g, neg);
-      if (!d) continue;
-      const uint32_t key = msm_bucket_key(a.g, k, w, d);
-      if (key != 0xffffffffu) f(key, (uint32_t)((uint64_t)w * a.g.point_stride + i) | (neg << 31));
-    }
+PB_HD void sort_digits(const SortArgs& a, const Fr& s, uint64_t i, uint32_t k, F f) {
+  DigitWalk dw(s);
+  for (uint32_t w = 0; w < a.g.W; w++) {
+    uint32_t neg, d = dw.next(w, a.g, neg);
+    if (!d) continue;
+    const uint32_t key = msm_bucket_key(a.g, k, w, d);
+    if (key != 0xffffffffu) f(key, (uint32_t)((uint64_t)w * a.g.point_stride + i) | (neg << 31));
+  }
+}
+
+template <class G>
+PB_HD void sort_walk(const SortArgs& a, uint32_t bx, uint32_t k, uint32_t t, uint32_t nt, G g) {
+  const uint64_t first = (uint64_t)bx * a.spb;
+  const uint64_t end = first + a.spb < a.n ? first + a.spb : a.n;
+  for (uint64_t i = first + t; i < end; i += nt) {
+    const Fr s = a.from_mont ? fp_from_mont(a.sb.p[k][i]) : a.sb.p[k][i];
+    g((uint32_t)(i - first), s);
   }
 }
 
 PB_HD void bin_hist(const SortArgs& a, uint32_t bx, uint32_t k, uint32_t t, uint32_t nt, uint32_t* sh_cnt) {
-  sort_walk(a, bx, k, t, nt, [&](uint32_t key, uint32_t) { sort_add(&sh_cnt[key >> a.lb], 1u); });
+  sort_walk(a, bx, k, t, nt, [&](uint32_t, const Fr& s) {
+    sort_digits(a, s, 0, k, [&](uint32_t key, uint32_t) { sort_add(&sh_cnt[key >> a.lb], 1u); });
+  });
 }
 
 PB_HD void bin_flush(const SortArgs& a, uint32_t t, uint32_t nt, const uint32_t* sh_cnt) {
@@ -83,49 +110,141 @@
     if (sh_cnt[b]) sort_add(&a.bin_cnt[b], sh_cnt[b]);
 }
 
-PB_HD void bin_reserve(const SortArgs& a, uint32_t t, uint32_t nt, uint32_t run, uint32_t* sh_cnt, uint32_t* sh_loc,
-                       uint32_t* sh_base) {
+PB_HD uint32_t bin_chunks(const SortArgs& a, uint32_t cnt) {
+  return a.pad || cnt > a.T ? (cnt + a.T - 1) / a.T : 0;
+}
+
+PB_HD void bin_scan_sums(const SortArgs& a, uint32_t t, uint32_t nt, uint32_t& entries, uint32_t& chunks) {
+  const uint32_t per = (a.nbins + nt - 1) / nt;
+  entries = chunks = 0;
+  for (uint32_t b = t * per; b < t * per + per && b < a.nbins; b++) {
+    entries += a.bin_cnt[b];
+    chunks += bin_chunks(a, a.bin_cnt[b]);
+  }
+}
+
+PB_HD void bin_scan_write(const SortArgs& a, uint32_t t, uint32_t nt, uint32_t run_e, uint32_t run_c,
+                          uint32_t total_e, uint32_t total_c) {
+  const uint32_t per = (a.nbins + nt - 1) / nt;
+  for (uint32_t b = t * per; b < t * per + per && b < a.nbins; b++) {
+    const uint32_t c = a.bin_cnt[b];
+    a.bin_off[b] = run_e;
+    a.chunk_first[b] = run_c;
+    run_e += c;
+    run_c += bin_chunks(a, c);
+    a.bin_cnt[b] = 0;
+  }
+  if (t == 0) {
+    a.bin_off[a.nbins] = total_e;
+    a.chunk_first[a.nbins] = total_c;
+    if (!a.pad) a.offsets[a.g.nb] = total_e;
+  }
+}
+
+PB_HD void scatter_hist(const SortArgs& a, uint32_t bx, uint32_t k, uint32_t t, uint32_t nt, uint32_t* sh_cnt,
+                        Fr* sh_sc) {
+  sort_walk(a, bx, k, t, nt, [&](uint32_t j, const Fr& s) {
+    sh_sc[j] = s;
+    sort_digits(a, s, 0, k, [&](uint32_t key, uint32_t) { sort_add(&sh_cnt[key >> a.lb], 1u); });
+  });
+}
+
+PB_HD void scatter_reserve(const SortArgs& a, uint32_t t, uint32_t nt, uint32_t run, uint32_t* sh_cnt,
+                           uint32_t* sh_delta) {
   const uint32_t per = (a.nbins + nt - 1) / nt;
   for (uint32_t b = t * per; b < t * per + per && b < a.nbins; b++) {
     const uint32_t c = sh_cnt[b];
-    sh_loc[b] = run;
+    if (c) sh_delta[b] = a.bin_off[b] + sort_add(&a.bin_cnt[b], c) - run;
+    sh_cnt[b] = run;
     run += c;
-    if (c) sh_base[b] = a.bin_off[b] + sort_add(&a.bin_cnt[b], c);
-    sh_cnt[b] = 0;
-  }
-}
-
-PB_HD void bin_stage(const SortArgs& a, uint32_t bx, uint32_t k, uint32_t t, uint32_t nt, uint32_t* sh_cnt,
-                     const uint32_t* sh_loc, SortEntry* stage) {
-  sort_walk(a, bx, k, t, nt, [&](uint32_t key, uint32_t val) {
-    const uint32_t b = key >> a.lb;
-    SortEntry e;
-    e.key = key;
-    e.val = val;
-    stage[sh_loc[b] + sort_add(&sh_cnt[b], 1u)] = e;
-  });
-}
-
-PB_HD void bin_copy_out(const SortArgs& a, uint32_t t, uint32_t nt, uint32_t total, const uint32_t* sh_loc,
-                        const uint32_t* sh_base, const SortEntry* stage) {
+  }
+}
+
+PB_HD void scatter_stage(const SortArgs& a, uint32_t bx, uint32_t k, uint32_t t, uint32_t nt, uint32_t* sh_cnt,
+                         const Fr* sh_sc, SortEntry* stage) {
+  const uint64_t first = (uint64_t)bx * a.spb;
+  const uint32_t m = (uint32_t)(first + a.spb < a.n ? a.spb : a.n - first);
+  for (uint32_t j = t; j < m; j += nt)
+    sort_digits(a, sh_sc[j], first + j, k, [&](uint32_t key, uint32_t val) {
+      SortEntry e;
+      e.key = key;
+      e.val = val;
+      stage[sort_add(&sh_cnt[key >> a.lb], 1u)] = e;
+    });
+}
+
+PB_HD void scatter_copy_out(const SortArgs& a, uint32_t t, uint32_t nt, uint32_t total, const uint32_t* sh_delta,
+                            const SortEntry* stage) {
   for (uint32_t p = t; p < total; p += nt) {
     const SortEntry e = stage[p];
-    const uint32_t b = e.key >> a.lb;
-    a.binned[sh_base[b] + p - sh_loc[b]] = e;
-  }
-}
-
-PB_HD uint32_t chunk_map_sum(const SortArgs& a, uint32_t t) {
-  uint32_t s = 0;
-  for (uint32_t b = 8 * t; b < 8 * t + 8 && b < a.nbins; b++) s += (a.bin_cnt[b] + a.T - 1) / a.T;
+    a.binned[sh_delta[e.key >> a.lb] + p] = e;
+  }
+}
+
+struct SortBin {
+  uint32_t lo, hi;
+  uint32_t key0, nkeys;
+  bool heavy;
+};
+
+PB_HD SortBin sort_bin(const SortArgs& a, uint32_t b) {
+  SortBin s;
+  s.lo = a.bin_off[b];
+  s.hi = a.bin_off[b + 1];
+  s.key0 = b << a.lb;
+  s.nkeys = a.g.nb - s.key0 < (1u << a.lb) ? a.g.nb - s.key0 : 1u << a.lb;
+  s.heavy = s.hi - s.lo > a.T;
   return s;
 }
-PB_HD void chunk_map_write(const SortArgs& a, uint32_t t, uint32_t run, uint32_t total) {
-  for (uint32_t b = 8 * t; b < 8 * t + 8 && b < a.nbins; b++) {
-    a.chunk_first[b] = run;
-    run += (a.bin_cnt[b] + a.T - 1) / a.T;
-  }
-  if (t == 0) a.chunk_first[a.nbins] = total;
+
+PB_HD void place_hist(const SortArgs& a, const SortBin& s, uint32_t t, uint32_t nt, uint32_t* sh_cnt,
+                      SortEntry* stage) {
+  if (s.heavy) {
+    for (uint32_t l = t; l < s.nkeys; l += nt) sh_cnt[l] = a.counts[s.key0 + l];
+    return;
+  }
+  for (uint32_t i = s.lo + t; i < s.hi; i += 4 * nt) {
+    SortEntry e[4];
+    for (uint32_t u = 0; u < 4; u++)
+      if (i + u * nt < s.hi) e[u] = a.binned[i + u * nt];
+    for (uint32_t u = 0; u < 4; u++)
+      if (i + u * nt < s.hi) {
+        const uint32_t l = e[u].key - s.key0;
+        e[u].key = l | (sort_add(&sh_cnt[l], 1u) << PB_SORT_KEY_BITS);
+        stage[i + u * nt - s.lo] = e[u];
+      }
+  }
+}
+
+PB_HD void place_reserve(const SortArgs& a, const SortBin& s, uint32_t t, uint32_t nt, uint32_t run,
+                         uint32_t* sh_cnt, uint32_t* sh_max) {
+  const uint32_t per = (s.nkeys + nt - 1) / nt;
+  uint32_t m = 0;
+  for (uint32_t l = t * per; l < t * per + per && l < s.nkeys; l++) {
+    const uint32_t c = sh_cnt[l];
+    a.offsets[s.key0 + l] = s.lo + run;
+    a.counts[s.key0 + l] = s.heavy ? 0 : c;
+    sh_cnt[l] = run;
+    run += c;
+    m = c > m ? c : m;
+  }
+  if (m) sort_max(sh_max, m);
+}
+
+PB_HD void place_stage(const SortArgs& a, const SortBin& s, uint32_t t, uint32_t nt, const uint32_t* sh_cnt,
+                       const uint32_t* sh_max, const SortEntry* stage, uint32_t* stage_vals) {
+  if (t == 0 && *sh_max) sort_max(&a.counts[a.g.nb], *sh_max);
+  if (s.heavy) return;
+  const uint32_t mask = (1u << PB_SORT_KEY_BITS) - 1;
+  for (uint32_t i = t; i < s.hi - s.lo; i += nt) {
+    const SortEntry e = stage[i];
+    stage_vals[sh_cnt[e.key & mask] + (e.key >> PB_SORT_KEY_BITS)] = e.val;
+  }
+}
+
+PB_HD void place_copy_out(const SortArgs& a, const SortBin& s, uint32_t t, uint32_t nt, const uint32_t* stage_vals) {
+  if (s.heavy) return;
+  for (uint32_t p = t; p < s.hi - s.lo; p += nt) a.sorted[s.lo + p] = stage_vals[p];
 }
 
 struct SortChunk {
```

Measured after the change: 21.14 (median of 6 runs). 1.02x the previous value.
